# zd11024/NaviLLM

Measured on NVIDIA H100. Metric: nav_steps_per_sec, higher is better.
Workload: dtype bf16

## Files before the change

### navillm_b200/csrc/gemm_bf16.cu

```cuda
#include "nv_common.cuh"
#include "nv_fp8.cuh"
#include "nv_host.h"

namespace nv {

constexpr uint32_t GEMM_BLOCK_M = 128;
constexpr uint32_t GEMM_BLOCK_K = 64;
constexpr uint32_t GEMM_THREADS = 288;
constexpr uint32_t GEMM_CONSUMERS = 256;
constexpr uint32_t GEMM_GROUP_M = 16;

enum GemmFlags : uint32_t {
  GEMM_ADD = 1u,
  GEMM_OUT_F32 = 2u,
  GEMM_NO_GU = 4u,
};

enum { EPI_PLAIN = 0, EPI_SWIGLU = 1, EPI_DSWIGLU = 2, EPI_ROPE = 3, EPI_ATTND = 4 };

struct EpiAux {
  void* aux;
  int64_t ld_aux;
  uint32_t F;
  float* dvec;
  const int* pos;
  const __nv_bfloat16* cos_t;
  const __nv_bfloat16* sin_t;
  uint32_t rope_cols;
  const int8_t* w_exp;
};

template <uint32_t BLOCK_N, uint32_t STAGES, typename WT = __nv_bfloat16>
struct GemmSmem {
  static constexpr bool kFp8 = sizeof(WT) == 1;
  static constexpr uint32_t THREADS = kFp8 ? GEMM_THREADS + 128 : GEMM_THREADS;
  static constexpr uint32_t A_BYTES = GEMM_BLOCK_M * GEMM_BLOCK_K * 2;
  static constexpr uint32_t B_BYTES = BLOCK_N * GEMM_BLOCK_K * sizeof(WT);
  static constexpr uint32_t STAGE_BYTES = A_BYTES + B_BYTES;
  static constexpr uint32_t CVT_BYTES = kFp8 ? BLOCK_N * GEMM_BLOCK_K * 2 : 0;
  static constexpr uint32_t CVT_OFF = STAGES * STAGE_BYTES;
  static constexpr uint32_t BAR_OFF = CVT_OFF + STAGES * CVT_BYTES;
  static constexpr uint32_t DYN_BYTES = BAR_OFF + (kFp8 ? 3 : 2) * STAGES * 8 + 1024;
  static_assert(CVT_OFF % 1024 == 0, "the expanded stages are 128-byte-swizzle atoms");
  static constexpr uint32_t ACC_LD = BLOCK_N + 4;
  static_assert(GEMM_BLOCK_M * ACC_LD * 4 <= BAR_OFF, "accumulator staging reuses the stage ring");
  static_assert(DYN_BYTES <= 232448, "shared memory per block");
};

__device__ __forceinline__ void tile_coords(uint32_t tile, uint32_t num_m, uint32_t num_n, uint32_t& m_blk,
                                            uint32_t& n_blk, uint32_t group_m = GEMM_GROUP_M) {
  const uint32_t group_size = group_m * num_n;
  const uint32_t g = tile / group_size;
  const uint32_t first_m = g * group_m;
  const uint32_t gm = min(num_m - first_m, group_m);
  const uint32_t r = tile - g * group_size;
  m_blk = first_m + r % gm;
  n_blk = r / gm;
}

__device__ __forceinline__ float silu_bf16(float g) { return bf16_round(g / (1.f + __expf(-g))); }

__device__ __forceinline__ void ld_acc32(const float* p, uint32_t (&v)[32]) {
#pragma unroll
  for (uint32_t j = 0; j < 32; j += 4) {
    const uint4 x = *reinterpret_cast<const uint4*>(p + j);
    v[j] = x.x; v[j + 1] = x.y; v[j + 2] = x.z; v[j + 3] = x.w;
  }
}

template <uint32_t BLOCK_N, uint32_t STAGES, bool A_MN, bool B_MN, int EPI, typename WT = __nv_bfloat16>
__global__ void __launch_bounds__(GemmSmem<BLOCK_N, STAGES, WT>::THREADS, 1)
gemm_bf16_wgmma(const __grid_constant__ CUtensorMap tmap_a, const __grid_constant__ CUtensorMap tmap_b,
                void* __restrict__ Cout, int64_t ldc, const __nv_bfloat16* __restrict__ addend, int64_t ld_add,
                uint32_t M, uint32_t N, uint32_t K, uint32_t flags, EpiAux ea) {
  using L = GemmSmem<BLOCK_N, STAGES, WT>;
  static_assert(EPI == EPI_PLAIN || BLOCK_N == 256, "fused epilogues use the 128 x 256 tile");
  static_assert(!L::kFp8 || (EPI == EPI_PLAIN && !A_MN && !B_MN && BLOCK_N <= 128),
                "fp8 weights: plain epilogue, K-major operands, 32- or 128-wide tiles");
  extern __shared__ uint8_t smem_raw[];
  uint8_t* smem = reinterpret_cast<uint8_t*>((reinterpret_cast<uintptr_t>(smem_raw) + 1023) & ~uintptr_t(1023));
  uint8_t* smem_a = smem;
  uint8_t* smem_b = smem + STAGES * L::A_BYTES;
  uint8_t* smem_cvt = smem + L::CVT_OFF;
  uint64_t* full_bar = reinterpret_cast<uint64_t*>(smem + L::BAR_OFF);
  uint64_t* empty_bar = full_bar + STAGES;
  uint64_t* cvt_bar = empty_bar + STAGES;

  const uint32_t warp = warp_id_uniform();
  constexpr uint32_t TILE_N = (EPI == EPI_SWIGLU) ? 128u : BLOCK_N;
  const uint32_t num_m = ceil_div_u32(M, GEMM_BLOCK_M);
  const uint32_t num_n = ceil_div_u32(N, TILE_N);
  const uint32_t num_kb = ceil_div_u32(K, GEMM_BLOCK_K);
  uint32_t m_blk, n_blk;
  tile_coords(blockIdx.x, num_m, num_n, m_blk, n_blk);

  if (threadIdx.x == 0) {
    for (uint32_t i = 0; i < STAGES; ++i) {
      mbar_init(&full_bar[i], 1);
      mbar_init(&empty_bar[i], L::kFp8 ? 2 + 128 : 2);
      if constexpr (L::kFp8) mbar_init(&cvt_bar[i], 128);
    }
    fence_mbar_init();
  }
  __syncthreads();

  if (warp == 8) {
    tma_prefetch_desc(&tmap_a);
    tma_prefetch_desc(&tmap_b);
    const int32_t m0 = m_blk * GEMM_BLOCK_M;
    uint32_t stage = 0, phase = 0;
    for (uint32_t kb = 0; kb < num_kb; ++kb) {
      mbar_wait(&empty_bar[stage], phase ^ 1);
      if (elect_one()) {
        mbar_arrive_expect_tx(&full_bar[stage], L::STAGE_BYTES);
        const int32_t k0 = kb * GEMM_BLOCK_K;
        uint8_t* sa = smem_a + stage * L::A_BYTES;
        uint8_t* sb = smem_b + stage * L::B_BYTES;
        if constexpr (!A_MN) {
          tma_load_2d(sa, &tmap_a, &full_bar[stage], k0, m0);
        } else {
#pragma unroll
          for (uint32_t i = 0; i < GEMM_BLOCK_M / 64; ++i)
            tma_load_2d(sa + i * (GEMM_BLOCK_K * 128), &tmap_a, &full_bar[stage], m0 + i * 64, k0);
        }
        if constexpr (L::kFp8) {
          tma_load_2d(sb, &tmap_b, &full_bar[stage], k0, n_blk * BLOCK_N);
        } else if constexpr (!B_MN) {
          constexpr uint32_t BOX = BLOCK_N < 128 ? BLOCK_N : 128;
#pragma unroll
          for (uint32_t i = 0; i < BLOCK_N / BOX; ++i) {
            const int32_t n0 = (EPI == EPI_SWIGLU) ? (int32_t)(n_blk * 128 + i * ea.F) : (int32_t)(n_blk * BLOCK_N + i * BOX);
            tma_load_2d(sb + i * BOX * 128, &tmap_b, &full_bar[stage], k0, n0);
          }
        } else {
#pragma unroll
          for (uint32_t i = 0; i < BLOCK_N / 64; ++i)
            tma_load_2d(sb + i * (GEMM_BLOCK_K * 128), &tmap_b, &full_bar[stage], n_blk * BLOCK_N + i * 64, k0);
        }
      }
      __syncwarp();
      if (++stage == STAGES) { stage = 0; phase ^= 1; }
    }
    return;
  }

  if constexpr (L::kFp8) {
    if (warp >= 9) {
      constexpr uint32_t J = BLOCK_N * GEMM_BLOCK_K / 16 / 128;
      const uint32_t t = threadIdx.x - GEMM_THREADS;
      float scale[J];
#pragma unroll
      for (uint32_t j = 0; j < J; ++j) {
        const uint32_t n = n_blk * BLOCK_N + ((t + 128 * j) >> 2);
        scale[j] = n < N ? fp8_pow2(ea.w_exp[n]) : 1.f;
      }
      uint32_t stage = 0, phase = 0;
      for (uint32_t kb = 0; kb < num_kb; ++kb) {
        mbar_wait(&full_bar[stage], phase);
        const uint32_t src = smem_u32(smem_b + stage * L::B_BYTES);
        const uint32_t dst = smem_u32(smem_cvt + stage * L::CVT_BYTES);
#pragma unroll
        for (uint32_t j = 0; j < J; ++j) {
          const uint32_t q = t + 128 * j, row = q >> 2, c = q & 3;
          uint4 v;
          asm volatile("ld.shared.v4.b32 {%0, %1, %2, %3}, [%4];" : "=r"(v.x), "=r"(v.y), "=r"(v.z), "=r"(v.w) : "r"(src + q * 16));
          uint32_t o[8];
          fp8x4_to_bf16x4(v.x, scale[j], o[0], o[1]);
          fp8x4_to_bf16x4(v.y, scale[j], o[2], o[3]);
          fp8x4_to_bf16x4(v.z, scale[j], o[4], o[5]);
          fp8x4_to_bf16x4(v.w, scale[j], o[6], o[7]);
          sts128(dst + sw128_offset(row, 2 * c), o[0], o[1], o[2], o[3]);
          sts128(dst + sw128_offset(row, 2 * c + 1), o[4], o[5], o[6], o[7]);
        }
        fence_proxy_async_smem();
        mbar_arrive(&cvt_bar[stage]);
        mbar_arrive(&empty_bar[stage]);
        if (++stage == STAGES) { stage = 0; phase ^= 1; }
      }
      return;
    }
  }

  const uint32_t wg = warp >> 2;
  float acc[BLOCK_N / 2];
#pragma unroll
  for (uint32_t i = 0; i < BLOCK_N / 2; ++i) acc[i] = 0.f;
  {
    constexpr uint32_t A_KADV = A_MN ? (16 * 128) >> 4 : (16 * 2) >> 4;
    constexpr uint32_t B_KADV = B_MN ? (16 * 128) >> 4 : (16 * 2) >> 4;
    constexpr uint32_t A_LBO = A_MN ? GEMM_BLOCK_K * 128 : 0, B_LBO = B_MN ? GEMM_BLOCK_K * 128 : 0;
    uint32_t stage = 0, phase = 0, prev = 0;
    __builtin_assume(num_kb > 0);
    for (uint32_t kb = 0; kb < num_kb; ++kb) {
      mbar_wait(&full_bar[stage], phase);
      if constexpr (L::kFp8) mbar_wait(&cvt_bar[stage], phase);
      const uint64_t adesc = gmma_desc_sw128(smem_u32(smem_a + stage * L::A_BYTES + wg * 8192), A_LBO, 1024);
      const uint64_t bdesc = gmma_desc_sw128(smem_u32(L::kFp8 ? smem_cvt + stage * L::CVT_BYTES : smem_b + stage * L::B_BYTES),
                                             B_LBO, 1024);
      wgmma_fence();
#pragma unroll
      for (uint32_t k = 0; k < GEMM_BLOCK_K / 16; ++k)
        wgmma_ss_bf16<BLOCK_N, A_MN ? 1 : 0, B_MN ? 1 : 0>(acc, adesc + k * A_KADV, bdesc + k * B_KADV, 1u);
      wgmma_commit();
      wgmma_wait<1>();
      if (kb > 0 && (threadIdx.x & 127) == 0) mbar_arrive(&empty_bar[prev]);
      prev = stage;
      if (++stage == STAGES) { stage = 0; phase ^= 1; }
    }
    wgmma_wait<0>();
    reg_fence(acc);
  }

  float* acc_s = reinterpret_cast<float*>(smem);
  named_bar_sync(1, GEMM_CONSUMERS);
  {
    const uint32_t t = threadIdx.x & 127, lane = threadIdx.x & 31;
    const uint32_t r0 = wg * 64 + (t >> 5) * 16 + (lane >> 2);
#pragma unroll
    for (uint32_t i = 0; i < BLOCK_N / 8; ++i) {
      const uint32_t c = i * 8 + 2 * (lane & 3);
      *reinterpret_cast<float2*>(acc_s + r0 * L::ACC_LD + c) = make_float2(acc[4 * i], acc[4 * i + 1]);
      *reinterpret_cast<float2*>(acc_s + (r0 + 8) * L::ACC_LD + c) = make_float2(acc[4 * i + 2], acc[4 * i + 3]);
    }
  }
  named_bar_sync(1, GEMM_CONSUMERS);

  const uint32_t rl = threadIdx.x & 127, half = threadIdx.x >> 7;
  const uint32_t row = m_blk * GEMM_BLOCK_M + rl;
  const uint32_t col0 = n_blk * TILE_N;
  const float* arow = acc_s + rl * L::ACC_LD;
  if (row >= M) return;
  if constexpr (EPI == EPI_SWIGLU) {
    __nv_bfloat16* gu = reinterpret_cast<__nv_bfloat16*>(Cout) + static_cast<int64_t>(row) * ldc;
    __nv_bfloat16* hrow = reinterpret_cast<__nv_bfloat16*>(ea.aux) + static_cast<int64_t>(row) * ea.ld_aux;
#pragma unroll 1
    for (uint32_t c = half * 32; c < 128; c += 64) {
      uint32_t g[32], u[32];
      ld_acc32(arow + c, g);
      ld_acc32(arow + 128 + c, u);
      const uint32_t col = col0 + c;
      if (col < ea.F) {
#pragma unroll
        for (uint32_t j = 0; j < 32; j += 8) {
          uint4 og, ou, oh;
          uint32_t* pg = &og.x; uint32_t* pu = &ou.x; uint32_t* ph = &oh.x;
#pragma unroll
          for (uint32_t q = 0; q < 4; ++q) {
            pg[q] = pack_bf16x2(__uint_as_float(g[j + 2 * q]), __uint_as_float(g[j + 2 * q + 1]));
            pu[q] = pack_bf16x2(__uint_as_float(u[j + 2 * q]), __uint_as_float(u[j + 2 * q + 1]));
            ph[q] = pack_bf16x2(silu_bf16(bf16_lo(pg[q])) * bf16_lo(pu[q]), silu_bf16(bf16_hi(pg[q])) * bf16_hi(pu[q]));
          }
          if ((flags & GEMM_NO_GU) == 0) {
            *reinterpret_cast<uint4*>(gu + col + j) = og;
            *reinterpret_cast<uint4*>(gu + ea.F + col + j) = ou;
          }
          *reinterpret_cast<uint4*>(hrow + col + j) = oh;
        }
      }
    }
  } else if constexpr (EPI == EPI_DSWIGLU) {
    __nv_bfloat16* dgu = reinterpret_cast<__nv_bfloat16*>(Cout) + static_cast<int64_t>(row) * ldc;
    const __nv_bfloat16* gu = reinterpret_cast<const __nv_bfloat16*>(ea.aux) + static_cast<int64_t>(row) * ea.ld_aux;
#pragma unroll 1
    for (uint32_t c = half * 32; c < BLOCK_N; c += 64) {
      uint32_t v[32];
      ld_acc32(arow + c, v);
      const uint32_t col = col0 + c;
      if (col < ea.F) {
#pragma unroll
        for (uint32_t j = 0; j < 32; j += 8) {
          const uint4 gg = *reinterpret_cast<const uint4*>(gu + col + j);
          const uint4 uu = *reinterpret_cast<const uint4*>(gu + ea.F + col + j);
          const uint32_t* pg = &gg.x; const uint32_t* pu = &uu.x;
          uint4 og, ou;
          uint32_t* qg = &og.x; uint32_t* qu = &ou.x;
#pragma unroll
          for (uint32_t q = 0; q < 4; ++q) {
            float dg[2], du[2];
#pragma unroll
            for (uint32_t e = 0; e < 2; ++e) {
              const float d = bf16_round(__uint_as_float(v[j + 2 * q + e]));
              const float gv = e ? bf16_hi(pg[q]) : bf16_lo(pg[q]);
              const float uv = e ? bf16_hi(pu[q]) : bf16_lo(pu[q]);
              const float sg = 1.f / (1.f + __expf(-gv));
              dg[e] = d * uv * (sg * (1.f + gv * (1.f - sg)));
              du[e] = d * (gv * sg);
            }
            qg[q] = pack_bf16x2(dg[0], dg[1]);
            qu[q] = pack_bf16x2(du[0], du[1]);
          }
          *reinterpret_cast<uint4*>(dgu + col + j) = og;
          *reinterpret_cast<uint4*>(dgu + ea.F + col + j) = ou;
        }
      }
    }
  } else if constexpr (EPI == EPI_ROPE) {
    __nv_bfloat16* crow = reinterpret_cast<__nv_bfloat16*>(Cout) + static_cast<int64_t>(row) * ldc;
    const int p = ea.pos[row];
    const __nv_bfloat16* cs = ea.cos_t + static_cast<int64_t>(p) * 128;
    const __nv_bfloat16* sn = ea.sin_t + static_cast<int64_t>(p) * 128;
#pragma unroll 1
    for (uint32_t it = half; it < 4; it += 2) {
      const uint32_t hh = (it >> 1) * 128, c = (it & 1) * 32;
      uint32_t a[32], b[32];
      ld_acc32(arow + hh + c, a);
      ld_acc32(arow + hh + 64 + c, b);
      const uint32_t col = col0 + hh + c;
      if (col < N) {
        const bool rope = col < ea.rope_cols;
#pragma unroll
        for (uint32_t j = 0; j < 32; j += 8) {
          uint4 o1, o2;
          uint32_t* p1 = &o1.x; uint32_t* p2 = &o2.x;
          uint4 c1 = make_uint4(0, 0, 0, 0), s1 = c1, c2 = c1, s2 = c1;
          if (rope) {
            c1 = *reinterpret_cast<const uint4*>(cs + c + j);      s1 = *reinterpret_cast<const uint4*>(sn + c + j);
            c2 = *reinterpret_cast<const uint4*>(cs + 64 + c + j); s2 = *reinterpret_cast<const uint4*>(sn + 64 + c + j);
          }
          const uint32_t* pc1 = &c1.x; const uint32_t* ps1 = &s1.x; const uint32_t* pc2 = &c2.x; const uint32_t* ps2 = &s2.x;
#pragma unroll
          for (uint32_t q = 0; q < 4; ++q) {
            const uint32_t xa = pack_bf16x2(__uint_as_float(a[j + 2 * q]), __uint_as_float(a[j + 2 * q + 1]));
            const uint32_t xb = pack_bf16x2(__uint_as_float(b[j + 2 * q]), __uint_as_float(b[j + 2 * q + 1]));
            if (rope) {
              const float y1l = bf16_round(bf16_lo(xa) * bf16_lo(pc1[q])) + bf16_round(-bf16_lo(xb) * bf16_lo(ps1[q]));
              const float y1h = bf16_round(bf16_hi(xa) * bf16_hi(pc1[q])) + bf16_round(-bf16_hi(xb) * bf16_hi(ps1[q]));
              const float y2l = bf16_round(bf16_lo(xb) * bf16_lo(pc2[q])) + bf16_round(bf16_lo(xa) * bf16_lo(ps2[q]));
              const float y2h = bf16_round(bf16_hi(xb) * bf16_hi(pc2[q])) + bf16_round(bf16_hi(xa) * bf16_hi(ps2[q]));
              p1[q] = pack_bf16x2(y1l, y1h);
              p2[q] = pack_bf16x2(y2l, y2h);
            } else {
              p1[q] = xa;
              p2[q] = xb;
            }
          }
          *reinterpret_cast<uint4*>(crow + col + j) = o1;
          *reinterpret_cast<uint4*>(crow + col + 64 + j) = o2;
        }
      }
    }
  } else if constexpr (EPI == EPI_ATTND) {
    __nv_bfloat16* drow = reinterpret_cast<__nv_bfloat16*>(Cout) + static_cast<int64_t>(row) * ldc;
    const __nv_bfloat16* orow = reinterpret_cast<const __nv_bfloat16*>(ea.aux) + static_cast<int64_t>(row) * ea.ld_aux;
    const uint32_t hc = col0 + half * 128;
    if (hc < N) {
      float dsum = 0.f;
#pragma unroll 1
      for (uint32_t c = 0; c < 128; c += 32) {
        uint32_t v[32];
        ld_acc32(arow + half * 128 + c, v);
        const uint32_t col = hc + c;
#pragma unroll
        for (uint32_t j = 0; j < 32; j += 8) {
          uint4 o;
          o.x = pack_bf16x2(__uint_as_float(v[j + 0]), __uint_as_float(v[j + 1]));
          o.y = pack_bf16x2(__uint_as_float(v[j + 2]), __uint_as_float(v[j + 3]));
          o.z = pack_bf16x2(__uint_as_float(v[j + 4]), __uint_as_float(v[j + 5]));
          o.w = pack_bf16x2(__uint_as_float(v[j + 6]), __uint_as_float(v[j + 7]));
          const uint4 a = *reinterpret_cast<const uint4*>(orow + col + j);
          dsum += bf16_lo(o.x) * bf16_lo(a.x) + bf16_hi(o.x) * bf16_hi(a.x) + bf16_lo(o.y) * bf16_lo(a.y) + bf16_hi(o.y) * bf16_hi(a.y)
                + bf16_lo(o.z) * bf16_lo(a.z) + bf16_hi(o.z) * bf16_hi(a.z) + bf16_lo(o.w) * bf16_lo(a.w) + bf16_hi(o.w) * bf16_hi(a.w);
          *reinterpret_cast<uint4*>(drow + col + j) = o;
        }
      }
      ea.dvec[static_cast<int64_t>(hc >> 7) * M + row] = dsum;
    }
  } else {
    const bool do_add = (flags & GEMM_ADD) != 0;
    const bool out_f32 = (flags & GEMM_OUT_F32) != 0;
#pragma unroll 1
    for (uint32_t c = half * 32; c < BLOCK_N; c += 64) {
      uint32_t v[32];
      ld_acc32(arow + c, v);
      const uint32_t col = col0 + c;
      if (col >= N) break;
      if (out_f32) {
        float* dst = reinterpret_cast<float*>(Cout) + static_cast<int64_t>(row) * ldc + col;
        if (col + 32 <= N && (ldc & 3) == 0) {
#pragma unroll
          for (uint32_t j = 0; j < 32; j += 4)
            *reinterpret_cast<uint4*>(dst + j) = make_uint4(v[j], v[j + 1], v[j + 2], v[j + 3]);
        } else {
#pragma unroll
          for (uint32_t j = 0; j < 32; ++j)
            if (col + j < N) dst[j] = __uint_as_float(v[j]);
        }
      } else {
        __nv_bfloat16* dst = reinterpret_cast<__nv_bfloat16*>(Cout) + static_cast<int64_t>(row) * ldc + col;
        const __nv_bfloat16* add = do_add ? addend + static_cast<int64_t>(row) * ld_add + col : nullptr;
        if (col + 32 <= N && (ldc & 7) == 0 && (!do_add || (ld_add & 7) == 0)) {
#pragma unroll
          for (uint32_t j = 0; j < 32; j += 8) {
            uint4 o;
            o.x = pack_bf16x2(__uint_as_float(v[j + 0]), __uint_as_float(v[j + 1]));
            o.y = pack_bf16x2(__uint_as_float(v[j + 2]), __uint_as_float(v[j + 3]));
            o.z = pack_bf16x2(__uint_as_float(v[j + 4]), __uint_as_float(v[j + 5]));
            o.w = pack_bf16x2(__uint_as_float(v[j + 6]), __uint_as_float(v[j + 7]));
            if (do_add) {
              const uint4 a = *reinterpret_cast<const uint4*>(add + j);
              o.x = pack_bf16x2(bf16_lo(o.x) + bf16_lo(a.x), bf16_hi(o.x) + bf16_hi(a.x));
              o.y = pack_bf16x2(bf16_lo(o.y) + bf16_lo(a.y), bf16_hi(o.y) + bf16_hi(a.y));
              o.z = pack_bf16x2(bf16_lo(o.z) + bf16_lo(a.z), bf16_hi(o.z) + bf16_hi(a.z));
              o.w = pack_bf16x2(bf16_lo(o.w) + bf16_lo(a.w), bf16_hi(o.w) + bf16_hi(a.w));
            }
            *reinterpret_cast<uint4*>(dst + j) = o;
          }
        } else {
#pragma unroll
          for (uint32_t j = 0; j < 32; ++j) {
            if (col + j < N) {
              float x = bf16_round(__uint_as_float(v[j]));
              if (do_add) x = x + __bfloat162float(add[j]);
              dst[j] = __float2bfloat16_rn(x);
            }
          }
        }
      }
    }
  }
}

template <uint32_t BN, uint32_t ST, bool A_MN, bool B_MN, int EPI = EPI_PLAIN, typename WT = __nv_bfloat16>
static int launch_gemm(const CUtensorMap& ta, const CUtensorMap& tb, void* C, int64_t ldc, const void* addend,
                       int64_t ld_add, uint32_t M, uint32_t N, uint32_t K, uint32_t flags, cudaStream_t stream,
                       EpiAux ea = EpiAux{}) {
  using L = GemmSmem<BN, ST, WT>;
  auto kern = gemm_bf16_wgmma<BN, ST, A_MN, B_MN, EPI, WT>;
  static bool attr_set = false;
  if (!attr_set) {
    NV_CUDA(cudaFuncSetAttribute(kern, cudaFuncAttributeMaxDynamicSharedMemorySize, L::DYN_BYTES));
    attr_set = true;
  }
  const uint32_t tiles = ceil_div_u32(M, GEMM_BLOCK_M) * ceil_div_u32(N, EPI == EPI_SWIGLU ? 128u : BN);
  kern<<<tiles, L::THREADS, L::DYN_BYTES, stream>>>(ta, tb, C, ldc, reinterpret_cast<const __nv_bfloat16*>(addend), ld_add,
                                                      M, N, K, flags, ea);
  NV_LAUNCH_CHECK();
  return NV_OK;
}

constexpr uint32_t WIDE_N = 256;
constexpr uint32_t WIDE_STAGES = 4;
constexpr uint32_t WIDE_CLUSTER = 2;

struct WideSmem {
  static constexpr uint32_t A_BYTES = GEMM_BLOCK_M * GEMM_BLOCK_K * 2;
  static constexpr uint32_t B_BYTES = WIDE_N * GEMM_BLOCK_K * 2;
  static constexpr uint32_t STAGE_BYTES = A_BYTES + B_BYTES;
  static constexpr uint32_t STG_OFF = WIDE_STAGES * STAGE_BYTES;
  static constexpr uint32_t STG_BYTES = GEMM_BLOCK_M * 128 * 2;
  static constexpr uint32_t BAR_OFF = STG_OFF + STG_BYTES;
  static constexpr uint32_t DYN_BYTES = BAR_OFF + 2 * WIDE_STAGES * 8 + 1024;
  static_assert(DYN_BYTES <= 232448, "shared memory per block");
};

__device__ __forceinline__ uint32_t stg_offset(uint32_t row, uint32_t chunk) {
  return row * 256u + ((chunk ^ (row & 7u)) << 4);
}
__device__ __forceinline__ int stg_chunk(uint32_t i, uint32_t p) {
  return ((i >> 3) & 1) == p ? int(i < 16 ? i - 8 * p : i - 8 - 8 * p) : -1;
}
__device__ __forceinline__ void ld_stg32(uint32_t stg, uint32_t row, uint32_t chunk, uint32_t (&w)[16]) {
#pragma unroll
  for (uint32_t q = 0; q < 4; ++q) {
    const uint4 x = lds128(stg + stg_offset(row, chunk + q));
    w[4 * q] = x.x; w[4 * q + 1] = x.y; w[4 * q + 2] = x.z; w[4 * q + 3] = x.w;
  }
}

__device__ __forceinline__ void store_plain32(const uint32_t (&w)[16], void* Cout, int64_t ldc, const __nv_bfloat16* addend,
                                              int64_t ld_add, uint32_t row, uint32_t col, uint32_t N, bool do_add) {
  if (col >= N) return;
  __nv_bfloat16* dst = reinterpret_cast<__nv_bfloat16*>(Cout) + static_cast<int64_t>(row) * ldc + col;
  const __nv_bfloat16* add = do_add ? addend + static_cast<int64_t>(row) * ld_add + col : nullptr;
  if (col + 32 <= N && (ldc & 7) == 0 && (!do_add || (ld_add & 7) == 0)) {
#pragma unroll
    for (uint32_t j = 0; j < 4; ++j) {
      uint4 o = make_uint4(w[4 * j], w[4 * j + 1], w[4 * j + 2], w[4 * j + 3]);
      if (do_add) {
        const uint4 a = *reinterpret_cast<const uint4*>(add + 8 * j);
        o.x = pack_bf16x2(bf16_lo(o.x) + bf16_lo(a.x), bf16_hi(o.x) + bf16_hi(a.x));
        o.y = pack_bf16x2(bf16_lo(o.y) + bf16_lo(a.y), bf16_hi(o.y) + bf16_hi(a.y));
        o.z = pack_bf16x2(bf16_lo(o.z) + bf16_lo(a.z), bf16_hi(o.z) + bf16_hi(a.z));
        o.w = pack_bf16x2(bf16_lo(o.w) + bf16_lo(a.w), bf16_hi(o.w) + bf16_hi(a.w));
      }
      *reinterpret_cast<uint4*>(dst + 8 * j) = o;
    }
  } else {
#pragma unroll
    for (uint32_t j = 0; j < 32; ++j) {
      if (col + j < N) {
        float x = (j & 1) ? bf16_hi(w[j >> 1]) : bf16_lo(w[j >> 1]);
        if (do_add) x = x + __bfloat162float(add[j]);
        dst[j] = __float2bfloat16_rn(x);
      }
    }
  }
}

template <bool A_MN, bool B_MN>
__global__ void __launch_bounds__(GEMM_THREADS, 1)
gemm_bf16_wide(const __grid_constant__ CUtensorMap tmap_a, const __grid_constant__ CUtensorMap tmap_b,
               void* __restrict__ Cout, int64_t ldc, const __nv_bfloat16* __restrict__ addend, int64_t ld_add,
               uint32_t M, uint32_t N, uint32_t K, uint32_t flags) {
  using L = WideSmem;
  extern __shared__ uint8_t smem_raw[];
  uint8_t* smem = reinterpret_cast<uint8_t*>((reinterpret_cast<uintptr_t>(smem_raw) + 1023) & ~uintptr_t(1023));
  uint8_t* smem_a = smem;
  uint8_t* smem_b = smem + WIDE_STAGES * L::A_BYTES;
  const uint32_t stg = smem_u32(smem + L::STG_OFF);
  uint64_t* full_bar = reinterpret_cast<uint64_t*>(smem + L::BAR_OFF);
  uint64_t* empty_bar = full_bar + WIDE_STAGES;

  const uint32_t warp = warp_id_uniform();
  const uint32_t rank = cluster_ctarank();
  const uint32_t pair = blockIdx.x / WIDE_CLUSTER;
  const uint32_t num_m = ceil_div_u32(M, GEMM_BLOCK_M);
  const uint32_t num_mp = ceil_div_u32(num_m, WIDE_CLUSTER);
  const uint32_t num_n = ceil_div_u32(N, WIDE_N);
  const uint32_t num_kb = ceil_div_u32(K, GEMM_BLOCK_K);

  if (threadIdx.x == 0) {
    for (uint32_t i = 0; i < WIDE_STAGES; ++i) {
      mbar_init(&full_bar[i], 1);
      mbar_init(&empty_bar[i], 2 * WIDE_CLUSTER);
    }
    fence_mbar_init();
  }
  cluster_sync_all();

  uint32_t mp, n_blk;
  tile_coords(pair, num_mp, num_n, mp, n_blk, GEMM_GROUP_M / WIDE_CLUSTER);
  const uint32_t m_blk = mp * WIDE_CLUSTER + rank;

  if (warp == 8) {
    tma_prefetch_desc(&tmap_a);
    tma_prefetch_desc(&tmap_b);
    uint32_t stage = 0, phase = 0;
    {
      const int32_t m0 = m_blk * GEMM_BLOCK_M;
      for (uint32_t kb = 0; kb < num_kb; ++kb) {
        mbar_wait(&empty_bar[stage], phase ^ 1);
        if (elect_one()) {
          mbar_arrive_expect_tx(&full_bar[stage], L::STAGE_BYTES);
          const int32_t k0 = kb * GEMM_BLOCK_K;
          uint8_t* sa = smem_a + stage * L::A_BYTES;
          uint8_t* sb = smem_b + stage * L::B_BYTES;
          if constexpr (!A_MN) {
            tma_load_2d(sa, &tmap_a, &full_bar[stage], k0, m0);
          } else {
#pragma unroll
            for (uint32_t i = 0; i < GEMM_BLOCK_M / 64; ++i)
              tma_load_2d(sa + i * (GEMM_BLOCK_K * 128), &tmap_a, &full_bar[stage], m0 + i * 64, k0);
          }
          constexpr uint32_t BOXES = B_MN ? WIDE_N / 64 : 2, BOX_BYTES = L::B_BYTES / BOXES;
#pragma unroll
          for (uint32_t j = 0; j < BOXES / WIDE_CLUSTER; ++j) {
            const uint32_t i = rank * (BOXES / WIDE_CLUSTER) + j;
            int32_t c0, c1;
            if constexpr (B_MN) { c0 = n_blk * WIDE_N + i * 64; c1 = k0; }
            else { c0 = k0; c1 = n_blk * WIDE_N + i * 128; }
            tma_load_2d_multicast(sb + i * BOX_BYTES, &tmap_b, &full_bar[stage], c0, c1, (1u << WIDE_CLUSTER) - 1);
          }
        }
        __syncwarp();
        if (++stage == WIDE_STAGES) { stage = 0; phase ^= 1; }
      }
    }
  } else {
    const uint32_t wg = warp >> 2, t = threadIdx.x & 127, lane = threadIdx.x & 31;
    const uint32_t r0 = wg * 64 + (t >> 5) * 16 + (lane >> 2);
    constexpr uint32_t A_KADV = A_MN ? (16 * 128) >> 4 : (16 * 2) >> 4;
    constexpr uint32_t B_KADV = B_MN ? (16 * 128) >> 4 : (16 * 2) >> 4;
    constexpr uint32_t A_LBO = A_MN ? GEMM_BLOCK_K * 128 : 0, B_LBO = B_MN ? GEMM_BLOCK_K * 128 : 0;
    const bool do_add = (flags & GEMM_ADD) != 0;
    uint32_t stage = 0, phase = 0;
    {
      float acc[WIDE_N / 2];
#pragma unroll
      for (uint32_t i = 0; i < WIDE_N / 2; ++i) acc[i] = 0.f;
      uint32_t prev = 0;
      for (uint32_t kb = 0; kb < num_kb; ++kb) {
        mbar_wait(&full_bar[stage], phase);
        const uint64_t adesc = gmma_desc_sw128(smem_u32(smem_a + stage * L::A_BYTES + wg * 8192), A_LBO, 1024);
        const uint64_t bdesc = gmma_desc_sw128(smem_u32(smem_b + stage * L::B_BYTES), B_LBO, 1024);
        wgmma_fence();
#pragma unroll
        for (uint32_t k = 0; k < GEMM_BLOCK_K / 16; ++k)
          wgmma_ss_bf16<WIDE_N, A_MN ? 1 : 0, B_MN ? 1 : 0>(acc, adesc + k * A_KADV, bdesc + k * B_KADV, 1u);
        wgmma_commit();
        wgmma_wait<1>();
        if (kb > 0 && t == 0)
          for (uint32_t c = 0; c < WIDE_CLUSTER; ++c) mbar_arrive_cluster(&empty_bar[prev], c);
        prev = stage;
        if (++stage == WIDE_STAGES) { stage = 0; phase ^= 1; }
      }
      wgmma_wait<0>();
      reg_fence(acc);

      const uint32_t row = m_blk * GEMM_BLOCK_M + t;
      const uint32_t col0 = n_blk * WIDE_N;
#pragma unroll
      for (uint32_t p = 0; p < 2; ++p) {
        named_bar_sync(1, GEMM_CONSUMERS);
#pragma unroll
        for (uint32_t i = 0; i < WIDE_N / 8; ++i) {
          const int sc = stg_chunk(i, p);
          if (sc < 0) continue;
          sts32(stg + stg_offset(r0, sc) + 4 * (lane & 3), pack_bf16x2(acc[4 * i], acc[4 * i + 1]));
          sts32(stg + stg_offset(r0 + 8, sc) + 4 * (lane & 3), pack_bf16x2(acc[4 * i + 2], acc[4 * i + 3]));
        }
        named_bar_sync(1, GEMM_CONSUMERS);
        if (row >= M) continue;
#pragma unroll 1
          for (uint32_t h = 0; h < 2; ++h) {
            uint32_t v[16];
            ld_stg32(stg, t, 8 * h + 4 * wg, v);
            store_plain32(v, Cout, ldc, addend, ld_add, row, col0 + 128 * h + 64 * p + 32 * wg, N, do_add);
          }
      }
    }
  }
  __syncwarp();
  cluster_sync_all();
}

template <bool A_MN, bool B_MN>
static int launch_wide(const CUtensorMap& ta, const CUtensorMap& tb, void* C, int64_t ldc, const void* addend,
                       int64_t ld_add, uint32_t M, uint32_t N, uint32_t K, uint32_t flags, cudaStream_t stream) {
  auto kern = gemm_bf16_wide<A_MN, B_MN>;
  cudaLaunchConfig_t cfg = {};
  cfg.blockDim = dim3(GEMM_THREADS);
  cfg.dynamicSmemBytes = WideSmem::DYN_BYTES;
  cfg.stream = stream;
  cudaLaunchAttribute attr[1];
  attr[0].id = cudaLaunchAttributeClusterDimension;
  attr[0].val.clusterDim.x = WIDE_CLUSTER;
  attr[0].val.clusterDim.y = 1;
  attr[0].val.clusterDim.z = 1;
  cfg.attrs = attr;
  cfg.numAttrs = 1;
  static bool attr_set = false;
  if (!attr_set) {
    NV_CUDA(cudaFuncSetAttribute(kern, cudaFuncAttributeMaxDynamicSharedMemorySize, WideSmem::DYN_BYTES));
    attr_set = true;
  }
  const uint32_t pairs = ceil_div_u32(ceil_div_u32(M, GEMM_BLOCK_M), WIDE_CLUSTER) * ceil_div_u32(N, WIDE_N);
  cfg.gridDim = dim3(WIDE_CLUSTER * pairs);
  NV_CUDA(cudaLaunchKernelEx(&cfg, kern, ta, tb, C, ldc, reinterpret_cast<const __nv_bfloat16*>(addend), ld_add, M, N, K,
                             flags));
  return NV_OK;
}

static int gemm_tmaps(CUtensorMap* ta, CUtensorMap* tb, const void* A, int64_t lda, int a_mn, const void* B, int64_t ldb,
                      int b_mn, int M, int N, int K, uint32_t block_n, uint64_t b_rows) {
  int rc;
  if (!a_mn) rc = make_tmap_2d(ta, A, 2, (uint64_t)K, (uint64_t)M, (uint64_t)lda * 2, 64, GEMM_BLOCK_M);
  else       rc = make_tmap_2d(ta, A, 2, (uint64_t)M, (uint64_t)K, (uint64_t)lda * 2, 64, GEMM_BLOCK_K);
  if (rc) return rc;
  if (!b_mn) rc = make_tmap_2d(tb, B, 2, (uint64_t)K, b_rows, (uint64_t)ldb * 2, 64, block_n < 128 ? block_n : 128);
  else       rc = make_tmap_2d(tb, B, 2, (uint64_t)N, (uint64_t)K, (uint64_t)ldb * 2, 64, GEMM_BLOCK_K);
  return rc;
}

}

extern "C" int nv_gemm_bf16(const void* A, int64_t lda, int a_mn, const void* B, int64_t ldb, int b_mn, void* C,
                            int64_t ldc, const void* addend, int64_t ld_add, int M, int N, int K, unsigned flags,
                            int block_n, void* stream_) {
  using namespace nv;
  cudaStream_t stream = reinterpret_cast<cudaStream_t>(stream_);
  NV_REQUIRE(M > 0 && N > 0 && K > 0, "nv_gemm_bf16: empty problem M=%d N=%d K=%d", M, N, K);
  NV_REQUIRE(A && B && C, "nv_gemm_bf16: null operand");
  NV_REQUIRE(!(flags & GEMM_ADD) || addend, "nv_gemm_bf16: GEMM_ADD without addend");
  NV_REQUIRE(!((flags & GEMM_ADD) && (flags & GEMM_OUT_F32)), "nv_gemm_bf16: ADD with fp32 output unsupported");
  NV_REQUIRE((lda & 7) == 0 && (ldb & 7) == 0, "nv_gemm_bf16: lda/ldb must be multiples of 8 (got %lld, %lld)",
             (long long)lda, (long long)ldb);
  if (block_n == 0) {
    const long wide_tiles = ((long)(M + 127) / 128) * ((long)(N + 255) / 256);
    block_n = (wide_tiles >= sm_count() && M >= 512) ? 256 : 128;
    if (M <= 128 && !a_mn && !b_mn) block_n = N <= 4096 ? 32 : 128;
  }
  NV_REQUIRE(block_n == 32 || block_n == 128 || block_n == 256, "nv_gemm_bf16: block_n must be 32, 128 or 256");
  NV_REQUIRE(!(block_n == 32 && b_mn), "nv_gemm_bf16: block_n = 32 (skinny-M weight streaming) needs a K-major B");

  if (block_n == 256 && (flags & GEMM_OUT_F32)) block_n = 128;

  CUtensorMap ta, tb;
  int rc = gemm_tmaps(&ta, &tb, A, lda, a_mn, B, ldb, b_mn, M, N, K, (uint32_t)block_n, (uint64_t)N);
  if (rc) return rc;

  if (block_n == 256) {
    if (!a_mn && !b_mn) return launch_wide<false, false>(ta, tb, C, ldc, addend, ld_add, M, N, K, flags, stream);
    if (!a_mn && b_mn) return launch_wide<false, true>(ta, tb, C, ldc, addend, ld_add, M, N, K, flags, stream);
    if (a_mn && b_mn) return launch_wide<true, true>(ta, tb, C, ldc, addend, ld_add, M, N, K, flags, stream);
    return launch_wide<true, false>(ta, tb, C, ldc, addend, ld_add, M, N, K, flags, stream);
  }

#define NV_GEMM_CASE(BN, ST)                                                                                       \
  do {                                                                                                             \
    if (!a_mn && !b_mn) return launch_gemm<BN, ST, false, false>(ta, tb, C, ldc, addend, ld_add, M, N, K, flags, stream); \
    if (!a_mn && b_mn) return launch_gemm<BN, ST, false, true>(ta, tb, C, ldc, addend, ld_add, M, N, K, flags, stream);   \
    if (a_mn && b_mn) return launch_gemm<BN, ST, true, true>(ta, tb, C, ldc, addend, ld_add, M, N, K, flags, stream);     \
    return launch_gemm<BN, ST, true, false>(ta, tb, C, ldc, addend, ld_add, M, N, K, flags, stream);                      \
  } while (0)

  if (block_n == 32) {
    if (!a_mn) return launch_gemm<32, 10, false, false>(ta, tb, C, ldc, addend, ld_add, M, N, K, flags, stream);
    return launch_gemm<32, 10, true, false>(ta, tb, C, ldc, addend, ld_add, M, N, K, flags, stream);
  }
  NV_GEMM_CASE(128, 6);
#undef NV_GEMM_CASE
}

extern "C" int nv_gemm_fp8w_bf16(const void* A, int64_t lda, const void* Wq, int64_t ldw, const void* exps, void* C, int64_t ldc,
                                 const void* addend, int64_t ld_add, int M, int N, int K, int block_n, void* stream_) {
  using namespace nv;
  cudaStream_t stream = reinterpret_cast<cudaStream_t>(stream_);
  NV_REQUIRE(M > 0 && N > 0 && K > 0, "nv_gemm_fp8w_bf16: empty problem M=%d N=%d K=%d", M, N, K);
  NV_REQUIRE(A && Wq && exps && C, "nv_gemm_fp8w_bf16: null operand");
  NV_REQUIRE((lda & 7) == 0 && (ldw & 15) == 0,
             "nv_gemm_fp8w_bf16: lda must be a multiple of 8 and ldw (bytes) of 16 (got %lld, %lld)", (long long)lda, (long long)ldw);
  if (block_n == 0) block_n = (M <= 128 && N <= 4096) ? 32 : 128;
  NV_REQUIRE(block_n == 32 || block_n == 128, "nv_gemm_fp8w_bf16: block_n must be 0, 32 or 128 (got %d)", block_n);
  CUtensorMap ta, tb;
  int rc = make_tmap_2d(&ta, A, 2, (uint64_t)K, (uint64_t)M, (uint64_t)lda * 2, 64, GEMM_BLOCK_M);
  if (rc) return rc;
  if ((rc = make_tmap_2d(&tb, Wq, 1, (uint64_t)K, (uint64_t)N, (uint64_t)ldw, 64, (uint32_t)block_n, false)))
    return rc;
  EpiAux ea{};
  ea.w_exp = reinterpret_cast<const int8_t*>(exps);
  const uint32_t flags = addend ? GEMM_ADD : 0u;
  if (block_n == 32)
    return launch_gemm<32, 10, false, false, EPI_PLAIN, uint8_t>(ta, tb, C, ldc, addend, ld_add, M, N, K, flags, stream, ea);
  return launch_gemm<128, 5, false, false, EPI_PLAIN, uint8_t>(ta, tb, C, ldc, addend, ld_add, M, N, K, flags, stream, ea);
}

extern "C" {

int nv_gemm_swiglu_bf16(const void* x, int64_t ldx, const void* Wgu, int64_t ldw, void* gu, int64_t ldgu, void* h,
                        int64_t ldh, int M, int F, int K, int keep_gu, void* stream) {
  using namespace nv;
  NV_REQUIRE(M > 0 && F > 0 && K > 0 && (F % 128) == 0, "nv_gemm_swiglu_bf16: F must be a multiple of 128 (got %d)", F);
  NV_REQUIRE((ldx & 7) == 0 && (ldw & 7) == 0 && (ldgu & 7) == 0 && (ldh & 7) == 0, "nv_gemm_swiglu_bf16: alignment");
  CUtensorMap ta, tb;
  int rc = gemm_tmaps(&ta, &tb, x, ldx, 0, Wgu, ldw, 0, M, 2 * F, K, 256, (uint64_t)2 * F);
  if (rc) return rc;
  EpiAux ea{};
  ea.aux = h; ea.ld_aux = ldh; ea.F = (uint32_t)F;
  return launch_gemm<256, 4, false, false, EPI_SWIGLU>(ta, tb, gu, ldgu, nullptr, 0, M, F, K, keep_gu ? 0u : GEMM_NO_GU,
                                                       reinterpret_cast<cudaStream_t>(stream), ea);
}

int nv_gemm_dswiglu_bf16(const void* dx, int64_t lddx, const void* Wd, int64_t ldw, const void* gu, int64_t ldgu, void* dgu,
                         int64_t lddgu, int M, int F, int D, void* stream) {
  using namespace nv;
  NV_REQUIRE(M > 0 && F > 0 && D > 0 && (F % 32) == 0, "nv_gemm_dswiglu_bf16: F %% 32");
  NV_REQUIRE((lddx & 7) == 0 && (ldw & 7) == 0 && (ldgu & 7) == 0 && (lddgu & 7) == 0, "nv_gemm_dswiglu_bf16: alignment");
  CUtensorMap ta, tb;
  int rc = gemm_tmaps(&ta, &tb, dx, lddx, 0, Wd, ldw, 1, M, F, D, 256, (uint64_t)F);
  if (rc) return rc;
  EpiAux ea{};
  ea.aux = const_cast<void*>(gu); ea.ld_aux = ldgu; ea.F = (uint32_t)F;
  return launch_gemm<256, 4, false, true, EPI_DSWIGLU>(ta, tb, dgu, lddgu, nullptr, 0, M, F, D, 0u,
                                                       reinterpret_cast<cudaStream_t>(stream), ea);
}

int nv_gemm_attnd_bf16(const void* dy, int64_t lddy, const void* Wo, int64_t ldw, const void* o, int64_t ldo, void* dout,
                       int64_t lddo, float* dvec, int M, int D, int Dout, void* stream) {
  using namespace nv;
  NV_REQUIRE(M > 0 && D > 0 && Dout > 0 && (D % 128) == 0 && o && dvec, "nv_gemm_attnd_bf16: D %% 128 and O / dvec required");
  NV_REQUIRE((lddy & 7) == 0 && (ldw & 7) == 0 && (ldo & 7) == 0 && (lddo & 7) == 0, "nv_gemm_attnd_bf16: alignment");
  CUtensorMap ta, tb;
  int rc = gemm_tmaps(&ta, &tb, dy, lddy, 0, Wo, ldw, 1, M, D, Dout, 256, (uint64_t)D);
  if (rc) return rc;
  EpiAux ea{};
  ea.aux = const_cast<void*>(o); ea.ld_aux = ldo; ea.dvec = dvec;
  return launch_gemm<256, 4, false, true, EPI_ATTND>(ta, tb, dout, lddo, nullptr, 0, M, D, Dout, 0u,
                                                     reinterpret_cast<cudaStream_t>(stream), ea);
}

int nv_gemm_rope_bf16(const void* x, int64_t ldx, const void* W, int64_t ldw, void* out, int64_t ldo, const int* pos,
                      const void* cos_t, const void* sin_t, int M, int N, int K, int rope_cols, void* stream) {
  using namespace nv;
  NV_REQUIRE(M > 0 && N > 0 && K > 0 && (N % 128) == 0 && (rope_cols % 128) == 0, "nv_gemm_rope_bf16: head alignment");
  NV_REQUIRE((ldx & 7) == 0 && (ldw & 7) == 0 && (ldo & 7) == 0, "nv_gemm_rope_bf16: alignment");
  CUtensorMap ta, tb;
  int rc = gemm_tmaps(&ta, &tb, x, ldx, 0, W, ldw, 0, M, N, K, 256, (uint64_t)N);
  if (rc) return rc;
  EpiAux ea{};
  ea.pos = pos; ea.cos_t = reinterpret_cast<const __nv_bfloat16*>(cos_t); ea.sin_t = reinterpret_cast<const __nv_bfloat16*>(sin_t);
  ea.rope_cols = (uint32_t)rope_cols;
  return launch_gemm<256, 4, false, false, EPI_ROPE>(ta, tb, out, ldo, nullptr, 0, M, N, K, 0u,
                                                     reinterpret_cast<cudaStream_t>(stream), ea);
}

}
```

### navillm_b200/csrc/nv_common.cuh

```cuda
#pragma once

#include <cuda.h>
#include <cuda_bf16.h>
#include <cuda_runtime.h>
#include <stdint.h>
#include <stdio.h>

#include "nv_wgmma.cuh"

namespace nv {

__device__ __forceinline__ uint32_t smem_u32(const void* p) {
  return static_cast<uint32_t>(__cvta_generic_to_shared(p));
}
__device__ __forceinline__ uint32_t lane_id() {
  uint32_t l;
  asm volatile("mov.u32 %0, %%laneid;" : "=r"(l));
  return l;
}
__host__ __device__ constexpr uint32_t ceil_div_u32(uint32_t a, uint32_t b) { return (a + b - 1) / b; }

__device__ __forceinline__ uint32_t pack_bf16x2(float a, float b) {
  __nv_bfloat162 v = __floats2bfloat162_rn(a, b);
  return *reinterpret_cast<uint32_t*>(&v);
}
__device__ __forceinline__ float bf16_lo(uint32_t v) { return __uint_as_float(v << 16); }
__device__ __forceinline__ float bf16_hi(uint32_t v) { return __uint_as_float(v & 0xffff0000u); }
__device__ __forceinline__ float bf16_round(float x) { return __bfloat162float(__float2bfloat16_rn(x)); }

__device__ __forceinline__ void griddep_wait() { asm volatile("griddepcontrol.wait;" ::: "memory"); }
__device__ __forceinline__ void griddep_launch() { asm volatile("griddepcontrol.launch_dependents;" ::: "memory"); }

__device__ __forceinline__ void sts128(uint32_t saddr, uint32_t a, uint32_t b, uint32_t c, uint32_t d) {
  asm volatile("st.shared.v4.b32 [%0], {%1, %2, %3, %4};" ::"r"(saddr), "r"(a), "r"(b), "r"(c), "r"(d) : "memory");
}
__device__ __forceinline__ void sts32(uint32_t saddr, uint32_t a) {
  asm volatile("st.shared.b32 [%0], %1;" ::"r"(saddr), "r"(a) : "memory");
}
__device__ __forceinline__ uint4 lds128(uint32_t saddr) {
  uint4 v;
  asm volatile("ld.shared.v4.b32 {%0, %1, %2, %3}, [%4];" : "=r"(v.x), "=r"(v.y), "=r"(v.z), "=r"(v.w) : "r"(saddr) : "memory");
  return v;
}
__device__ __forceinline__ uint2 lds64(uint32_t saddr) {
  uint2 v;
  asm volatile("ld.shared.v2.b32 {%0, %1}, [%2];" : "=r"(v.x), "=r"(v.y) : "r"(saddr) : "memory");
  return v;
}

__device__ __forceinline__ void mbar_init(uint64_t* bar, uint32_t count) {
  asm volatile("mbarrier.init.shared::cta.b64 [%0], %1;" ::"r"(smem_u32(bar)), "r"(count) : "memory");
}
__device__ __forceinline__ void fence_mbar_init() {
  asm volatile("fence.mbarrier_init.release.cluster;" ::: "memory");
}
__device__ __forceinline__ void mbar_arrive(uint64_t* bar) {
  asm volatile("mbarrier.arrive.shared::cta.b64 _, [%0];" ::"r"(smem_u32(bar)) : "memory");
}
__device__ __forceinline__ void mbar_arrive_expect_tx(uint64_t* bar, uint32_t bytes) {
  asm volatile("mbarrier.arrive.expect_tx.shared::cta.b64 _, [%0], %1;" ::"r"(smem_u32(bar)), "r"(bytes)
               : "memory");
}
__device__ __forceinline__ bool mbar_try_wait(uint64_t* bar, uint32_t parity) {
  uint32_t ok;
  asm volatile(
      "{\n\t.reg .pred p;\n\t"
      "mbarrier.try_wait.parity.shared::cta.b64 p, [%1], %2;\n\t"
      "selp.u32 %0, 1, 0, p;\n\t}"
      : "=r"(ok)
      : "r"(smem_u32(bar)), "r"(parity)
      : "memory");
  return ok != 0;
}
#ifndef NV_MBAR_TIMEOUT_CYCLES
#define NV_MBAR_TIMEOUT_CYCLES (4000000000ll)
#endif
__device__ __forceinline__ void mbar_wait(uint64_t* bar, uint32_t parity) {
  if (mbar_try_wait(bar, parity)) return;
  const long long t0 = clock64();
  uint32_t spins = 0;
  while (!mbar_try_wait(bar, parity)) {
    if ((++spins & 255u) == 0 && clock64() - t0 > NV_MBAR_TIMEOUT_CYCLES) {
#ifdef NV_MBAR_TIMEOUT_REPORT
      printf("navillm_b200: mbarrier timeout block (%d,%d) thread %d bar@%u parity %u\n", (int)blockIdx.x,
             (int)blockIdx.y, (int)threadIdx.x, smem_u32(bar), parity);
#endif
      __trap();
    }
  }
}

__device__ __forceinline__ void fence_proxy_async_smem() {
  asm volatile("fence.proxy.async.shared::cta;" ::: "memory");
}

__device__ __forceinline__ void tma_prefetch_desc(const CUtensorMap* m) {
  asm volatile("prefetch.tensormap [%0];" ::"l"(reinterpret_cast<uint64_t>(m)) : "memory");
}
__device__ __forceinline__ void tma_load_2d(void* smem_dst, const CUtensorMap* m, uint64_t* bar, int32_t c0,
                                            int32_t c1) {
  asm volatile(
      "cp.async.bulk.tensor.2d.shared::cluster.global.mbarrier::complete_tx::bytes [%0], [%1, {%3, %4}], [%2];"
      ::"r"(smem_u32(smem_dst)), "l"(reinterpret_cast<uint64_t>(m)), "r"(smem_u32(bar)), "r"(c0), "r"(c1)
      : "memory");
}
__device__ __forceinline__ void tma_load_2d_multicast(void* smem_dst, const CUtensorMap* m, uint64_t* bar, int32_t c0,
                                                      int32_t c1, uint16_t cta_mask) {
  asm volatile(
      "cp.async.bulk.tensor.2d.shared::cluster.global.mbarrier::complete_tx::bytes.multicast::cluster"
      " [%0], [%1, {%3, %4}], [%2], %5;"
      ::"r"(smem_u32(smem_dst)), "l"(reinterpret_cast<uint64_t>(m)), "r"(smem_u32(bar)), "r"(c0), "r"(c1), "h"(cta_mask)
      : "memory");
}
__device__ __forceinline__ void tma_load_3d(void* smem_dst, const CUtensorMap* m, uint64_t* bar, int32_t c0,
                                            int32_t c1, int32_t c2) {
  asm volatile(
      "cp.async.bulk.tensor.3d.shared::cluster.global.mbarrier::complete_tx::bytes [%0], [%1, {%3, %4, %5}], [%2];"
      ::"r"(smem_u32(smem_dst)), "l"(reinterpret_cast<uint64_t>(m)), "r"(smem_u32(bar)), "r"(c0), "r"(c1), "r"(c2)
      : "memory");
}
__device__ __forceinline__ void tma_store_2d(const CUtensorMap* m, const void* smem_src, int32_t c0, int32_t c1) {
  asm volatile("cp.async.bulk.tensor.2d.global.shared::cta.bulk_group [%0, {%2, %3}], [%1];" ::"l"(
                   reinterpret_cast<uint64_t>(m)),
               "r"(smem_u32(smem_src)), "r"(c0), "r"(c1)
               : "memory");
}
__device__ __forceinline__ void tma_store_commit() { asm volatile("cp.async.bulk.commit_group;" ::: "memory"); }
template <int N>
__device__ __forceinline__ void tma_store_wait_read() {
  asm volatile("cp.async.bulk.wait_group.read %0;" ::"n"(N) : "memory");
}
template <int N>
__device__ __forceinline__ void tma_store_wait_all() {
  asm volatile("cp.async.bulk.wait_group %0;" ::"n"(N) : "memory");
}

__device__ __forceinline__ void wgmma_fence() { asm volatile("wgmma.fence.sync.aligned;" ::: "memory"); }
__device__ __forceinline__ void wgmma_commit() { asm volatile("wgmma.commit_group.sync.aligned;" ::: "memory"); }
template <int N>
__device__ __forceinline__ void wgmma_wait() {
  asm volatile("wgmma.wait_group.sync.aligned %0;" ::"n"(N) : "memory");
}
template <int R>
__device__ __forceinline__ void reg_fence(float (&d)[R]) {
#pragma unroll
  for (int i = 0; i < R; ++i) asm volatile("" : "+f"(d[i])::"memory");
}

__device__ __forceinline__ bool elect_one() {
  uint32_t pred;
  asm volatile("{\n\t.reg .pred e;\n\telect.sync _|e, 0xffffffff;\n\tselp.u32 %0, 1, 0, e;\n\t}" : "=r"(pred));
  return pred != 0;
}
__device__ __forceinline__ uint32_t warp_id_uniform() { return __shfl_sync(0xffffffffu, threadIdx.x >> 5, 0); }

__device__ __forceinline__ void named_bar_sync(uint32_t id, uint32_t count) {
  asm volatile("bar.sync %0, %1;" ::"r"(id), "r"(count) : "memory");
}

__device__ __forceinline__ void cluster_sync_all() {
  asm volatile("barrier.cluster.arrive.release.aligned;\n\tbarrier.cluster.wait.acquire.aligned;" ::: "memory");
}
__device__ __forceinline__ uint32_t cluster_ctarank() {
  uint32_t r;
  asm volatile("mov.u32 %0, %%cluster_ctarank;" : "=r"(r));
  return r;
}
__device__ __forceinline__ void mbar_arrive_cluster(uint64_t* bar, uint32_t cta) {
  asm volatile(
      "{\n\t.reg .b32 ra;\n\t"
      "mapa.shared::cluster.u32 ra, %0, %1;\n\t"
      "mbarrier.arrive.shared::cluster.b64 _, [ra];\n\t}"
      ::"r"(smem_u32(bar)), "r"(cta)
      : "memory");
}
__device__ __forceinline__ void dsmem_add_f32(uint32_t saddr, uint32_t cta, float v) {
  asm volatile(
      "{\n\t.reg .b32 ra;\n\t.reg .f32 x;\n\t"
      "mapa.shared::cluster.u32 ra, %0, %1;\n\t"
      "ld.shared::cluster.f32 x, [ra];\n\t"
      "add.f32 x, x, %2;\n\t"
      "st.shared::cluster.f32 [ra], x;\n\t}"
      ::"r"(saddr), "r"(cta), "f"(v)
      : "memory");
}

__device__ __forceinline__ uint64_t gmma_desc_sw128(uint32_t smem_addr, uint32_t lbo_bytes, uint32_t sbo_bytes) {
  uint64_t d = 0;
  d |= static_cast<uint64_t>((smem_addr >> 4) & 0x3FFFu);
  d |= static_cast<uint64_t>((lbo_bytes >> 4) & 0x3FFFu) << 16;
  d |= static_cast<uint64_t>((sbo_bytes >> 4) & 0x3FFFu) << 32;
  d |= static_cast<uint64_t>(1) << 62;
  return d;
}

__device__ __forceinline__ uint32_t sw128_offset(uint32_t row, uint32_t chunk) {
  return row * 128u + ((chunk ^ (row & 7u)) << 4);
}

}
```

Measured before the change: 22.23.

## Move fused SwiGLU/dSwiGLU/RoPE/attn-backward epilogues onto the clustered wide GEMM kernel

Removes the fused-epilogue variants from the simple 128x256 wgmma kernel and reimplements them in the clustered wide GEMM kernel. The new epilogues stage outputs in recycled pipeline smem slots with swizzled layouts and write them with TMA stores through per-epilogue tensor maps, and they also TMA-prefetch the auxiliary operands (gu, o). The goal is to give the fused MLP and attention-backward GEMMs the faster wide mainloop and to replace strided per-thread global stores and loads with bulk TMA traffic. This adds complexity in smem slot reuse and barrier handling, and there is risk of correctness issues in the swizzled epilogue indexing.

```diff
diff --git a/navillm_b200/csrc/gemm_bf16.cu b/navillm_b200/csrc/gemm_bf16.cu
--- a/navillm_b200/csrc/gemm_bf16.cu
+++ b/navillm_b200/csrc/gemm_bf16.cu
@@ -19,8 +19,6 @@
 enum { EPI_PLAIN = 0, EPI_SWIGLU = 1, EPI_DSWIGLU = 2, EPI_ROPE = 3, EPI_ATTND = 4 };
 
 struct EpiAux {
-  void* aux;
-  int64_t ld_aux;
   uint32_t F;
   float* dvec;
   const int* pos;
@@ -68,15 +66,14 @@
   }
 }
 
-template <uint32_t BLOCK_N, uint32_t STAGES, bool A_MN, bool B_MN, int EPI, typename WT = __nv_bfloat16>
+template <uint32_t BLOCK_N, uint32_t STAGES, bool A_MN, bool B_MN, typename WT = __nv_bfloat16>
 __global__ void __launch_bounds__(GemmSmem<BLOCK_N, STAGES, WT>::THREADS, 1)
 gemm_bf16_wgmma(const __grid_constant__ CUtensorMap tmap_a, const __grid_constant__ CUtensorMap tmap_b,
                 void* __restrict__ Cout, int64_t ldc, const __nv_bfloat16* __restrict__ addend, int64_t ld_add,
                 uint32_t M, uint32_t N, uint32_t K, uint32_t flags, EpiAux ea) {
   using L = GemmSmem<BLOCK_N, STAGES, WT>;
-  static_assert(EPI == EPI_PLAIN || BLOCK_N == 256, "fused epilogues use the 128 x 256 tile");
-  static_assert(!L::kFp8 || (EPI == EPI_PLAIN && !A_MN && !B_MN && BLOCK_N <= 128),
-                "fp8 weights: plain epilogue, K-major operands, 32- or 128-wide tiles");
+  static_assert(BLOCK_N <= 128, "the 128 x 256 tile is gemm_bf16_wide");
+  static_assert(!L::kFp8 || (!A_MN && !B_MN), "fp8 weights: K-major operands");
   extern __shared__ uint8_t smem_raw[];
   uint8_t* smem = reinterpret_cast<uint8_t*>((reinterpret_cast<uintptr_t>(smem_raw) + 1023) & ~uintptr_t(1023));
   uint8_t* smem_a = smem;
@@ -87,9 +84,8 @@
   uint64_t* cvt_bar = empty_bar + STAGES;
 
   const uint32_t warp = warp_id_uniform();
-  constexpr uint32_t TILE_N = (EPI == EPI_SWIGLU) ? 128u : BLOCK_N;
   const uint32_t num_m = ceil_div_u32(M, GEMM_BLOCK_M);
-  const uint32_t num_n = ceil_div_u32(N, TILE_N);
+  const uint32_t num_n = ceil_div_u32(N, BLOCK_N);
   const uint32_t num_kb = ceil_div_u32(K, GEMM_BLOCK_K);
   uint32_t m_blk, n_blk;
   tile_coords(blockIdx.x, num_m, num_n, m_blk, n_blk);
@@ -129,8 +125,7 @@
           constexpr uint32_t BOX = BLOCK_N < 128 ? BLOCK_N : 128;
 #pragma unroll
           for (uint32_t i = 0; i < BLOCK_N / BOX; ++i) {
-            const int32_t n0 = (EPI == EPI_SWIGLU) ? (int32_t)(n_blk * 128 + i * ea.F) : (int32_t)(n_blk * BLOCK_N + i * BOX);
-            tma_load_2d(sb + i * BOX * 128, &tmap_b, &full_bar[stage], k0, n0);
+            tma_load_2d(sb + i * BOX * 128, &tmap_b, &full_bar[stage], k0, n_blk * BLOCK_N + i * BOX);
           }
         } else {
 #pragma unroll
@@ -227,129 +222,32 @@
 
   const uint32_t rl = threadIdx.x & 127, half = threadIdx.x >> 7;
   const uint32_t row = m_blk * GEMM_BLOCK_M + rl;
-  const uint32_t col0 = n_blk * TILE_N;
+  const uint32_t col0 = n_blk * BLOCK_N;
   const float* arow = acc_s + rl * L::ACC_LD;
   if (row >= M) return;
-  if constexpr (EPI == EPI_SWIGLU) {
-    __nv_bfloat16* gu = reinterpret_cast<__nv_bfloat16*>(Cout) + static_cast<int64_t>(row) * ldc;
-    __nv_bfloat16* hrow = reinterpret_cast<__nv_bfloat16*>(ea.aux) + static_cast<int64_t>(row) * ea.ld_aux;
+  const bool do_add = (flags & GEMM_ADD) != 0;
+  const bool out_f32 = (flags & GEMM_OUT_F32) != 0;
 #pragma unroll 1
-    for (uint32_t c = half * 32; c < 128; c += 64) {
-      uint32_t g[32], u[32];
-      ld_acc32(arow + c, g);
-      ld_acc32(arow + 128 + c, u);
-      const uint32_t col = col0 + c;
-      if (col < ea.F) {
-#pragma unroll
-        for (uint32_t j = 0; j < 32; j += 8) {
-          uint4 og, ou, oh;
-          uint32_t* pg = &og.x; uint32_t* pu = &ou.x; uint32_t* ph = &oh.x;
-#pragma unroll
-          for (uint32_t q = 0; q < 4; ++q) {
-            pg[q] = pack_bf16x2(__uint_as_float(g[j + 2 * q]), __uint_as_float(g[j + 2 * q + 1]));
-            pu[q] = pack_bf16x2(__uint_as_float(u[j + 2 * q]), __uint_as_float(u[j + 2 * q + 1]));
-            ph[q] = pack_bf16x2(silu_bf16(bf16_lo(pg[q])) * bf16_lo(pu[q]), silu_bf16(bf16_hi(pg[q])) * bf16_hi(pu[q]));
-          }
-          if ((flags & GEMM_NO_GU) == 0) {
-            *reinterpret_cast<uint4*>(gu + col + j) = og;
-            *reinterpret_cast<uint4*>(gu + ea.F + col + j) = ou;
-          }
-          *reinterpret_cast<uint4*>(hrow + col + j) = oh;
-        }
-      }
-    }
-  } else if constexpr (EPI == EPI_DSWIGLU) {
-    __nv_bfloat16* dgu = reinterpret_cast<__nv_bfloat16*>(Cout) + static_cast<int64_t>(row) * ldc;
-    const __nv_bfloat16* gu = reinterpret_cast<const __nv_bfloat16*>(ea.aux) + static_cast<int64_t>(row) * ea.ld_aux;
-#pragma unroll 1
-    for (uint32_t c = half * 32; c < BLOCK_N; c += 64) {
-      uint32_t v[32];
-      ld_acc32(arow + c, v);
-      const uint32_t col = col0 + c;
-      if (col < ea.F) {
-#pragma unroll
-        for (uint32_t j = 0; j < 32; j += 8) {
-          const uint4 gg = *reinterpret_cast<const uint4*>(gu + col + j);
-          const uint4 uu = *reinterpret_cast<const uint4*>(gu + ea.F + col + j);
-          const uint32_t* pg = &gg.x; const uint32_t* pu = &uu.x;
-          uint4 og, ou;
-          uint32_t* qg = &og.x; uint32_t* qu = &ou.x;
-#pragma unroll
-          for (uint32_t q = 0; q < 4; ++q) {
-            float dg[2], du[2];
-#pragma unroll
-            for (uint32_t e = 0; e < 2; ++e) {
-              const float d = bf16_round(__uint_as_float(v[j + 2 * q + e]));
-              const float gv = e ? bf16_hi(pg[q]) : bf16_lo(pg[q]);
-              const float uv = e ? bf16_hi(pu[q]) : bf16_lo(pu[q]);
-              const float sg = 1.f / (1.f + __expf(-gv));
-              dg[e] = d * uv * (sg * (1.f + gv * (1.f - sg)));
-              du[e] = d * (gv * sg);
-            }
-            qg[q] = pack_bf16x2(dg[0], dg[1]);
-            qu[q] = pack_bf16x2(du[0], du[1]);
-          }
-          *reinterpret_cast<uint4*>(dgu + col + j) = og;
-          *reinterpret_cast<uint4*>(dgu + ea.F + col + j) = ou;
-        }
-      }
-    }
-  } else if constexpr (EPI == EPI_ROPE) {
-    __nv_bfloat16* crow = reinterpret_cast<__nv_bfloat16*>(Cout) + static_cast<int64_t>(row) * ldc;
-    const int p = ea.pos[row];
-    const __nv_bfloat16* cs = ea.cos_t + static_cast<int64_t>(p) * 128;
-    const __nv_bfloat16* sn = ea.sin_t + static_cast<int64_t>(p) * 128;
-#pragma unroll 1
-    for (uint32_t it = half; it < 4; it += 2) {
-      const uint32_t hh = (it >> 1) * 128, c = (it & 1) * 32;
-      uint32_t a[32], b[32];
-      ld_acc32(arow + hh + c, a);
-      ld_acc32(arow + hh + 64 + c, b);
-      const uint32_t col = col0 + hh + c;
-      if (col < N) {
-        const bool rope = col < ea.rope_cols;
-#pragma unroll
-        for (uint32_t j = 0; j < 32; j += 8) {
-          uint4 o1, o2;
-          uint32_t* p1 = &o1.x; uint32_t* p2 = &o2.x;
-          uint4 c1 = make_uint4(0, 0, 0, 0), s1 = c1, c2 = c1, s2 = c1;
-          if (rope) {
-            c1 = *reinterpret_cast<const uint4*>(cs + c + j);      s1 = *reinterpret_cast<const uint4*>(sn + c + j);
-            c2 = *reinterpret_cast<const uint4*>(cs + 64 + c + j); s2 = *reinterpret_cast<const uint4*>(sn + 64 + c + j);
-          }
-          const uint32_t* pc1 = &c1.x; const uint32_t* ps1 = &s1.x; const uint32_t* pc2 = &c2.x; const uint32_t* ps2 = &s2.x;
-#pragma unroll
-          for (uint32_t q = 0; q < 4; ++q) {
-            const uint32_t xa = pack_bf16x2(__uint_as_float(a[j + 2 * q]), __uint_as_float(a[j + 2 * q + 1]));
-            const uint32_t xb = pack_bf16x2(__uint_as_float(b[j + 2 * q]), __uint_as_float(b[j + 2 * q + 1]));
-            if (rope) {
-              const float y1l = bf16_round(bf16_lo(xa) * bf16_lo(pc1[q])) + bf16_round(-bf16_lo(xb) * bf16_lo(ps1[q]));
-              const float y1h = bf16_round(bf16_hi(xa) * bf16_hi(pc1[q])) + bf16_round(-bf16_hi(xb) * bf16_hi(ps1[q]));
-              const float y2l = bf16_round(bf16_lo(xb) * bf16_lo(pc2[q])) + bf16_round(bf16_lo(xa) * bf16_lo(ps2[q]));
-              const float y2h = bf16_round(bf16_hi(xb) * bf16_hi(pc2[q])) + bf16_round(bf16_hi(xa) * bf16_hi(ps2[q]));
-              p1[q] = pack_bf16x2(y1l, y1h);
-              p2[q] = pack_bf16x2(y2l, y2h);
-            } else {
-              p1[q] = xa;
-              p2[q] = xb;
-            }
-          }
-          *reinterpret_cast<uint4*>(crow + col + j) = o1;
-          *reinterpret_cast<uint4*>(crow + col + 64 + j) = o2;
-        }
-      }
-    }
-  } else if constexpr (EPI == EPI_ATTND) {
-    __nv_bfloat16* drow = reinterpret_cast<__nv_bfloat16*>(Cout) + static_cast<int64_t>(row) * ldc;
-    const __nv_bfloat16* orow = reinterpret_cast<const __nv_bfloat16*>(ea.aux) + static_cast<int64_t>(row) * ea.ld_aux;
-    const uint32_t hc = col0 + half * 128;
-    if (hc < N) {
-      float dsum = 0.f;
-#pragma unroll 1
-      for (uint32_t c = 0; c < 128; c += 32) {
-        uint32_t v[32];
-        ld_acc32(arow + half * 128 + c, v);
-        const uint32_t col = hc + c;
+  for (uint32_t c = half * 32; c < BLOCK_N; c += 64) {
+    uint32_t v[32];
+    ld_acc32(arow + c, v);
+    const uint32_t col = col0 + c;
+    if (col >= N) break;
+    if (out_f32) {
+      float* dst = reinterpret_cast<float*>(Cout) + static_cast<int64_t>(row) * ldc + col;
+      if (col + 32 <= N && (ldc & 3) == 0) {
+#pragma unroll
+        for (uint32_t j = 0; j < 32; j += 4)
+          *reinterpret_cast<uint4*>(dst + j) = make_uint4(v[j], v[j + 1], v[j + 2], v[j + 3]);
+      } else {
+#pragma unroll
+        for (uint32_t j = 0; j < 32; ++j)
+          if (col + j < N) dst[j] = __uint_as_float(v[j]);
+      }
+    } else {
+      __nv_bfloat16* dst = reinterpret_cast<__nv_bfloat16*>(Cout) + static_cast<int64_t>(row) * ldc + col;
+      const __nv_bfloat16* add = do_add ? addend + static_cast<int64_t>(row) * ld_add + col : nullptr;
+      if (col + 32 <= N && (ldc & 7) == 0 && (!do_add || (ld_add & 7) == 0)) {
 #pragma unroll
         for (uint32_t j = 0; j < 32; j += 8) {
           uint4 o;
@@ -357,81 +255,41 @@
           o.y = pack_bf16x2(__uint_as_float(v[j + 2]), __uint_as_float(v[j + 3]));
           o.z = pack_bf16x2(__uint_as_float(v[j + 4]), __uint_as_float(v[j + 5]));
           o.w = pack_bf16x2(__uint_as_float(v[j + 6]), __uint_as_float(v[j + 7]));
-          const uint4 a = *reinterpret_cast<const uint4*>(orow + col + j);
-          dsum += bf16_lo(o.x) * bf16_lo(a.x) + bf16_hi(o.x) * bf16_hi(a.x) + bf16_lo(o.y) * bf16_lo(a.y) + bf16_hi(o.y) * bf16_hi(a.y)
-                + bf16_lo(o.z) * bf16_lo(a.z) + bf16_hi(o.z) * bf16_hi(a.z) + bf16_lo(o.w) * bf16_lo(a.w) + bf16_hi(o.w) * bf16_hi(a.w);
-          *reinterpret_cast<uint4*>(drow + col + j) = o;
-        }
-      }
-      ea.dvec[static_cast<int64_t>(hc >> 7) * M + row] = dsum;
-    }
-  } else {
-    const bool do_add = (flags & GEMM_ADD) != 0;
-    const bool out_f32 = (flags & GEMM_OUT_F32) != 0;
-#pragma unroll 1
-    for (uint32_t c = half * 32; c < BLOCK_N; c += 64) {
-      uint32_t v[32];
-      ld_acc32(arow + c, v);
-      const uint32_t col = col0 + c;
-      if (col >= N) break;
-      if (out_f32) {
-        float* dst = reinterpret_cast<float*>(Cout) + static_cast<int64_t>(row) * ldc + col;
-        if (col + 32 <= N && (ldc & 3) == 0) {
-#pragma unroll
-          for (uint32_t j = 0; j < 32; j += 4)
-            *reinterpret_cast<uint4*>(dst + j) = make_uint4(v[j], v[j + 1], v[j + 2], v[j + 3]);
-        } else {
-#pragma unroll
-          for (uint32_t j = 0; j < 32; ++j)
-            if (col + j < N) dst[j] = __uint_as_float(v[j]);
+          if (do_add) {
+            const uint4 a = *reinterpret_cast<const uint4*>(add + j);
+            o.x = pack_bf16x2(bf16_lo(o.x) + bf16_lo(a.x), bf16_hi(o.x) + bf16_hi(a.x));
+            o.y = pack_bf16x2(bf16_lo(o.y) + bf16_lo(a.y), bf16_hi(o.y) + bf16_hi(a.y));
+            o.z = pack_bf16x2(bf16_lo(o.z) + bf16_lo(a.z), bf16_hi(o.z) + bf16_hi(a.z));
+            o.w = pack_bf16x2(bf16_lo(o.w) + bf16_lo(a.w), bf16_hi(o.w) + bf16_hi(a.w));
+          }
+          *reinterpret_cast<uint4*>(dst + j) = o;
         }
       } else {
-        __nv_bfloat16* dst = reinterpret_cast<__nv_bfloat16*>(Cout) + static_cast<int64_t>(row) * ldc + col;
-        const __nv_bfloat16* add = do_add ? addend + static_cast<int64_t>(row) * ld_add + col : nullptr;
-        if (col + 32 <= N && (ldc & 7) == 0 && (!do_add || (ld_add & 7) == 0)) {
-#pragma unroll
-          for (uint32_t j = 0; j < 32; j += 8) {
-            uint4 o;
-            o.x = pack_bf16x2(__uint_as_float(v[j + 0]), __uint_as_float(v[j + 1]));
-            o.y = pack_bf16x2(__uint_as_float(v[j + 2]), __uint_as_float(v[j + 3]));
-            o.z = pack_bf16x2(__uint_as_float(v[j + 4]), __uint_as_float(v[j + 5]));
-            o.w = pack_bf16x2(__uint_as_float(v[j + 6]), __uint_as_float(v[j + 7]));
-            if (do_add) {
-              const uint4 a = *reinterpret_cast<const uint4*>(add + j);
-              o.x = pack_bf16x2(bf16_lo(o.x) + bf16_lo(a.x), bf16_hi(o.x) + bf16_hi(a.x));
-              o.y = pack_bf16x2(bf16_lo(o.y) + bf16_lo(a.y), bf16_hi(o.y) + bf16_hi(a.y));
-              o.z = pack_bf16x2(bf16_lo(o.z) + bf16_lo(a.z), bf16_hi(o.z) + bf16_hi(a.z));
-              o.w = pack_bf16x2(bf16_lo(o.w) + bf16_lo(a.w), bf16_hi(o.w) + bf16_hi(a.w));
-            }
-            *reinterpret_cast<uint4*>(dst + j) = o;
+#pragma unroll
+        for (uint32_t j = 0; j < 32; ++j) {
+          if (col + j < N) {
+            float x = bf16_round(__uint_as_float(v[j]));
+            if (do_add) x = x + __bfloat162float(add[j]);
+            dst[j] = __float2bfloat16_rn(x);
           }
-        } else {
-#pragma unroll
-          for (uint32_t j = 0; j < 32; ++j) {
-            if (col + j < N) {
-              float x = bf16_round(__uint_as_float(v[j]));
-              if (do_add) x = x + __bfloat162float(add[j]);
-              dst[j] = __float2bfloat16_rn(x);
-            }
-          }
-        }
-      }
-    }
-  }
-}
-
-template <uint32_t BN, uint32_t ST, bool A_MN, bool B_MN, int EPI = EPI_PLAIN, typename WT = __nv_bfloat16>
+        }
+      }
+    }
+  }
+}
+
+template <uint32_t BN, uint32_t ST, bool A_MN, bool B_MN, typename WT = __nv_bfloat16>
 static int launch_gemm(const CUtensorMap& ta, const CUtensorMap& tb, void* C, int64_t ldc, const void* addend,
                        int64_t ld_add, uint32_t M, uint32_t N, uint32_t K, uint32_t flags, cudaStream_t stream,
                        EpiAux ea = EpiAux{}) {
   using L = GemmSmem<BN, ST, WT>;
-  auto kern = gemm_bf16_wgmma<BN, ST, A_MN, B_MN, EPI, WT>;
+  auto kern = gemm_bf16_wgmma<BN, ST, A_MN, B_MN, WT>;
   static bool attr_set = false;
   if (!attr_set) {
     NV_CUDA(cudaFuncSetAttribute(kern, cudaFuncAttributeMaxDynamicSharedMemorySize, L::DYN_BYTES));
     attr_set = true;
   }
-  const uint32_t tiles = ceil_div_u32(M, GEMM_BLOCK_M) * ceil_div_u32(N, EPI == EPI_SWIGLU ? 128u : BN);
+  const uint32_t tiles = ceil_div_u32(M, GEMM_BLOCK_M) * ceil_div_u32(N, BN);
   kern<<<tiles, L::THREADS, L::DYN_BYTES, stream>>>(ta, tb, C, ldc, reinterpret_cast<const __nv_bfloat16*>(addend), ld_add,
                                                       M, N, K, flags, ea);
   NV_LAUNCH_CHECK();
@@ -449,7 +307,7 @@
   static constexpr uint32_t STG_OFF = WIDE_STAGES * STAGE_BYTES;
   static constexpr uint32_t STG_BYTES = GEMM_BLOCK_M * 128 * 2;
   static constexpr uint32_t BAR_OFF = STG_OFF + STG_BYTES;
-  static constexpr uint32_t DYN_BYTES = BAR_OFF + 2 * WIDE_STAGES * 8 + 1024;
+  static constexpr uint32_t DYN_BYTES = BAR_OFF + (2 * WIDE_STAGES + 1) * 8 + 1024;
   static_assert(DYN_BYTES <= 232448, "shared memory per block");
 };
 
@@ -497,12 +355,32 @@
   }
 }
 
-template <bool A_MN, bool B_MN>
+constexpr uint32_t EPI_BOX_BYTES = GEMM_BLOCK_M * 128;
+
+struct EpiMaps {
+  CUtensorMap m[4];
+};
+
+__device__ __forceinline__ uint8_t* epi_slot(uint8_t* smem, uint32_t num_kb, uint32_t v) {
+  const uint32_t s = (num_kb + v / 3) % WIDE_STAGES, j = v % 3;
+  return j == 0 ? smem + s * WideSmem::A_BYTES
+                : smem + WIDE_STAGES * WideSmem::A_BYTES + s * WideSmem::B_BYTES + (j - 1) * EPI_BOX_BYTES;
+}
+__device__ __forceinline__ uint32_t frag_offset(uint32_t r, uint32_t i, uint32_t lane) {
+  return sw128_offset(r, i & 7) + 4 * (lane & 3);
+}
+
+template <bool A_MN, bool B_MN, int EPI>
 __global__ void __launch_bounds__(GEMM_THREADS, 1)
 gemm_bf16_wide(const __grid_constant__ CUtensorMap tmap_a, const __grid_constant__ CUtensorMap tmap_b,
-               void* __restrict__ Cout, int64_t ldc, const __nv_bfloat16* __restrict__ addend, int64_t ld_add,
-               uint32_t M, uint32_t N, uint32_t K, uint32_t flags) {
+               const __grid_constant__ EpiMaps em, void* __restrict__ Cout, int64_t ldc,
+               const __nv_bfloat16* __restrict__ addend, int64_t ld_add, uint32_t M, uint32_t N, uint32_t K,
+               uint32_t flags, EpiAux ea) {
   using L = WideSmem;
+  static_assert(EPI == EPI_PLAIN || (!A_MN && B_MN == (EPI == EPI_DSWIGLU || EPI == EPI_ATTND)),
+                "fused epilogues: the operand forms of their entry points");
+  constexpr uint32_t TILE_N = EPI == EPI_SWIGLU ? 128u : WIDE_N;
+  constexpr uint32_t PRE_BOXES = EPI == EPI_DSWIGLU ? 8 : EPI == EPI_ATTND ? 4 : 0;
   extern __shared__ uint8_t smem_raw[];
   uint8_t* smem = reinterpret_cast<uint8_t*>((reinterpret_cast<uintptr_t>(smem_raw) + 1023) & ~uintptr_t(1023));
   uint8_t* smem_a = smem;
@@ -510,13 +388,14 @@
   const uint32_t stg = smem_u32(smem + L::STG_OFF);
   uint64_t* full_bar = reinterpret_cast<uint64_t*>(smem + L::BAR_OFF);
   uint64_t* empty_bar = full_bar + WIDE_STAGES;
+  uint64_t* epi_full = empty_bar + WIDE_STAGES;
 
   const uint32_t warp = warp_id_uniform();
   const uint32_t rank = cluster_ctarank();
   const uint32_t pair = blockIdx.x / WIDE_CLUSTER;
   const uint32_t num_m = ceil_div_u32(M, GEMM_BLOCK_M);
   const uint32_t num_mp = ceil_div_u32(num_m, WIDE_CLUSTER);
-  const uint32_t num_n = ceil_div_u32(N, WIDE_N);
+  const uint32_t num_n = ceil_div_u32(N, TILE_N);
   const uint32_t num_kb = ceil_div_u32(K, GEMM_BLOCK_K);
 
   if (threadIdx.x == 0) {
@@ -524,6 +403,7 @@
       mbar_init(&full_bar[i], 1);
       mbar_init(&empty_bar[i], 2 * WIDE_CLUSTER);
     }
+    mbar_init(epi_full, 1);
     fence_mbar_init();
   }
   cluster_sync_all();
@@ -531,39 +411,55 @@
   uint32_t mp, n_blk;
   tile_coords(pair, num_mp, num_n, mp, n_blk, GEMM_GROUP_M / WIDE_CLUSTER);
   const uint32_t m_blk = mp * WIDE_CLUSTER + rank;
+  const int32_t m0 = m_blk * GEMM_BLOCK_M;
+  const uint32_t col0 = n_blk * TILE_N;
 
   if (warp == 8) {
     tma_prefetch_desc(&tmap_a);
     tma_prefetch_desc(&tmap_b);
     uint32_t stage = 0, phase = 0;
-    {
-      const int32_t m0 = m_blk * GEMM_BLOCK_M;
-      for (uint32_t kb = 0; kb < num_kb; ++kb) {
-        mbar_wait(&empty_bar[stage], phase ^ 1);
-        if (elect_one()) {
-          mbar_arrive_expect_tx(&full_bar[stage], L::STAGE_BYTES);
-          const int32_t k0 = kb * GEMM_BLOCK_K;
-          uint8_t* sa = smem_a + stage * L::A_BYTES;
-          uint8_t* sb = smem_b + stage * L::B_BYTES;
-          if constexpr (!A_MN) {
-            tma_load_2d(sa, &tmap_a, &full_bar[stage], k0, m0);
-          } else {
-#pragma unroll
-            for (uint32_t i = 0; i < GEMM_BLOCK_M / 64; ++i)
-              tma_load_2d(sa + i * (GEMM_BLOCK_K * 128), &tmap_a, &full_bar[stage], m0 + i * 64, k0);
+    for (uint32_t kb = 0; kb < num_kb; ++kb) {
+      mbar_wait(&empty_bar[stage], phase ^ 1);
+      if (elect_one()) {
+        mbar_arrive_expect_tx(&full_bar[stage], L::STAGE_BYTES);
+        const int32_t k0 = kb * GEMM_BLOCK_K;
+        uint8_t* sa = smem_a + stage * L::A_BYTES;
+        uint8_t* sb = smem_b + stage * L::B_BYTES;
+        if constexpr (!A_MN) {
+          tma_load_2d(sa, &tmap_a, &full_bar[stage], k0, m0);
+        } else {
+#pragma unroll
+          for (uint32_t i = 0; i < GEMM_BLOCK_M / 64; ++i)
+            tma_load_2d(sa + i * (GEMM_BLOCK_K * 128), &tmap_a, &full_bar[stage], m0 + i * 64, k0);
+        }
+        constexpr uint32_t BOXES = B_MN ? WIDE_N / 64 : 2, BOX_BYTES = L::B_BYTES / BOXES;
+#pragma unroll
+        for (uint32_t j = 0; j < BOXES / WIDE_CLUSTER; ++j) {
+          const uint32_t i = rank * (BOXES / WIDE_CLUSTER) + j;
+          int32_t c0, c1;
+          if constexpr (B_MN) { c0 = n_blk * WIDE_N + i * 64; c1 = k0; }
+          else { c0 = k0; c1 = EPI == EPI_SWIGLU ? col0 + i * ea.F : n_blk * WIDE_N + i * 128; }
+          tma_load_2d_multicast(sb + i * BOX_BYTES, &tmap_b, &full_bar[stage], c0, c1, (1u << WIDE_CLUSTER) - 1);
+        }
+      }
+      __syncwarp();
+      if (++stage == WIDE_STAGES) { stage = 0; phase ^= 1; }
+    }
+    if constexpr (PRE_BOXES > 0) {
+      if (m_blk < num_m) {
+        if (elect_one()) mbar_arrive_expect_tx(epi_full, PRE_BOXES * EPI_BOX_BYTES);
+        __syncwarp();
+#pragma unroll
+        for (uint32_t v0 = 0; v0 < PRE_BOXES; v0 += 3) {
+          mbar_wait(&empty_bar[stage], phase ^ 1);
+          if (elect_one()) {
+#pragma unroll
+            for (uint32_t v = v0; v < v0 + 3 && v < PRE_BOXES; ++v)
+              tma_load_2d(epi_slot(smem, num_kb, v), &em.m[2 + v / 4], epi_full, col0 + 64 * (v % 4), m0);
           }
-          constexpr uint32_t BOXES = B_MN ? WIDE_N / 64 : 2, BOX_BYTES = L::B_BYTES / BOXES;
-#pragma unroll
-          for (uint32_t j = 0; j < BOXES / WIDE_CLUSTER; ++j) {
-            const uint32_t i = rank * (BOXES / WIDE_CLUSTER) + j;
-            int32_t c0, c1;
-            if constexpr (B_MN) { c0 = n_blk * WIDE_N + i * 64; c1 = k0; }
-            else { c0 = k0; c1 = n_blk * WIDE_N + i * 128; }
-            tma_load_2d_multicast(sb + i * BOX_BYTES, &tmap_b, &full_bar[stage], c0, c1, (1u << WIDE_CLUSTER) - 1);
-          }
-        }
-        __syncwarp();
-        if (++stage == WIDE_STAGES) { stage = 0; phase ^= 1; }
+          __syncwarp();
+          if (++stage == WIDE_STAGES) { stage = 0; phase ^= 1; }
+        }
       }
     }
   } else {
@@ -572,13 +468,13 @@
     constexpr uint32_t A_KADV = A_MN ? (16 * 128) >> 4 : (16 * 2) >> 4;
     constexpr uint32_t B_KADV = B_MN ? (16 * 128) >> 4 : (16 * 2) >> 4;
     constexpr uint32_t A_LBO = A_MN ? GEMM_BLOCK_K * 128 : 0, B_LBO = B_MN ? GEMM_BLOCK_K * 128 : 0;
-    const bool do_add = (flags & GEMM_ADD) != 0;
     uint32_t stage = 0, phase = 0;
     {
       float acc[WIDE_N / 2];
 #pragma unroll
       for (uint32_t i = 0; i < WIDE_N / 2; ++i) acc[i] = 0.f;
       uint32_t prev = 0;
+      __builtin_assume(num_kb > 0);
       for (uint32_t kb = 0; kb < num_kb; ++kb) {
         mbar_wait(&full_bar[stage], phase);
         const uint64_t adesc = gmma_desc_sw128(smem_u32(smem_a + stage * L::A_BYTES + wg * 8192), A_LBO, 1024);
@@ -597,26 +493,153 @@
       wgmma_wait<0>();
       reg_fence(acc);
 
-      const uint32_t row = m_blk * GEMM_BLOCK_M + t;
-      const uint32_t col0 = n_blk * WIDE_N;
-#pragma unroll
-      for (uint32_t p = 0; p < 2; ++p) {
-        named_bar_sync(1, GEMM_CONSUMERS);
-#pragma unroll
-        for (uint32_t i = 0; i < WIDE_N / 8; ++i) {
-          const int sc = stg_chunk(i, p);
-          if (sc < 0) continue;
-          sts32(stg + stg_offset(r0, sc) + 4 * (lane & 3), pack_bf16x2(acc[4 * i], acc[4 * i + 1]));
-          sts32(stg + stg_offset(r0 + 8, sc) + 4 * (lane & 3), pack_bf16x2(acc[4 * i + 2], acc[4 * i + 3]));
-        }
-        named_bar_sync(1, GEMM_CONSUMERS);
-        if (row >= M) continue;
+      if constexpr (EPI == EPI_PLAIN) {
+        const bool do_add = (flags & GEMM_ADD) != 0;
+        const uint32_t row = m_blk * GEMM_BLOCK_M + t;
+#pragma unroll
+        for (uint32_t p = 0; p < 2; ++p) {
+          named_bar_sync(1, GEMM_CONSUMERS);
+#pragma unroll
+          for (uint32_t i = 0; i < WIDE_N / 8; ++i) {
+            const int sc = stg_chunk(i, p);
+            if (sc < 0) continue;
+            sts32(stg + stg_offset(r0, sc) + 4 * (lane & 3), pack_bf16x2(acc[4 * i], acc[4 * i + 1]));
+            sts32(stg + stg_offset(r0 + 8, sc) + 4 * (lane & 3), pack_bf16x2(acc[4 * i + 2], acc[4 * i + 3]));
+          }
+          named_bar_sync(1, GEMM_CONSUMERS);
+          if (row >= M) continue;
 #pragma unroll 1
           for (uint32_t h = 0; h < 2; ++h) {
             uint32_t v[16];
             ld_stg32(stg, t, 8 * h + 4 * wg, v);
             store_plain32(v, Cout, ldc, addend, ld_add, row, col0 + 128 * h + 64 * p + 32 * wg, N, do_add);
           }
+        }
+      } else {
+        named_bar_sync(1, GEMM_CONSUMERS);
+        if (m_blk < num_m) {
+          uint8_t* slot[8];
+#pragma unroll
+          for (uint32_t v = 0; v < 8; ++v) slot[v] = epi_slot(smem, num_kb, v);
+          constexpr uint32_t OUT_BOXES = EPI == EPI_SWIGLU ? 6 : EPI == EPI_DSWIGLU ? 8 : 4;
+          constexpr uint32_t OUT_SLOT0 = EPI == EPI_ATTND ? 4 : 0;
+          if constexpr (EPI == EPI_SWIGLU) {
+#pragma unroll
+            for (uint32_t i = 0; i < 16; ++i) {
+#pragma unroll
+              for (uint32_t h = 0; h < 2; ++h) {
+                const uint32_t g = pack_bf16x2(acc[4 * i + 2 * h], acc[4 * i + 2 * h + 1]);
+                const uint32_t u = pack_bf16x2(acc[4 * (i + 16) + 2 * h], acc[4 * (i + 16) + 2 * h + 1]);
+                const uint32_t off = frag_offset(r0 + 8 * h, i, lane);
+                sts32(smem_u32(slot[i / 8]) + off, g);
+                sts32(smem_u32(slot[2 + i / 8]) + off, u);
+                sts32(smem_u32(slot[4 + i / 8]) + off,
+                      pack_bf16x2(silu_bf16(bf16_lo(g)) * bf16_lo(u), silu_bf16(bf16_hi(g)) * bf16_hi(u)));
+              }
+            }
+          } else if constexpr (EPI == EPI_DSWIGLU) {
+            mbar_wait(epi_full, 0);
+#pragma unroll
+            for (uint32_t i = 0; i < 32; ++i) {
+#pragma unroll
+              for (uint32_t h = 0; h < 2; ++h) {
+                const uint32_t off = frag_offset(r0 + 8 * h, i, lane);
+                const uint32_t ga = smem_u32(slot[i / 8]) + off, ua = smem_u32(slot[4 + i / 8]) + off;
+                const uint32_t gp = lds32(ga), up = lds32(ua);
+                float dg[2], du[2];
+#pragma unroll
+                for (uint32_t e = 0; e < 2; ++e) {
+                  const float d = bf16_round(acc[4 * i + 2 * h + e]);
+                  const float gv = e ? bf16_hi(gp) : bf16_lo(gp);
+                  const float uv = e ? bf16_hi(up) : bf16_lo(up);
+                  const float sg = 1.f / (1.f + __expf(-gv));
+                  dg[e] = d * uv * (sg * (1.f + gv * (1.f - sg)));
+                  du[e] = d * (gv * sg);
+                }
+                sts32(ga, pack_bf16x2(dg[0], dg[1]));
+                sts32(ua, pack_bf16x2(du[0], du[1]));
+              }
+            }
+          } else if constexpr (EPI == EPI_ROPE) {
+            const bool rope0 = col0 < ea.rope_cols, rope1 = col0 + 128 < ea.rope_cols;
+            int p[2];
+#pragma unroll
+            for (uint32_t h = 0; h < 2; ++h) p[h] = m0 + r0 + 8 * h < M ? ea.pos[m0 + r0 + 8 * h] : 0;
+#pragma unroll
+            for (uint32_t i = 0; i < 8; ++i) {
+#pragma unroll
+              for (uint32_t h = 0; h < 2; ++h) {
+                const uint32_t c = 8 * i + 2 * (lane & 3), off = frag_offset(r0 + 8 * h, i, lane);
+                uint32_t c1 = 0, s1 = 0, c2 = 0, s2 = 0;
+                if (rope0) {
+                  const int64_t b = static_cast<int64_t>(p[h]) * 128 + c;
+                  c1 = *reinterpret_cast<const uint32_t*>(ea.cos_t + b);
+                  s1 = *reinterpret_cast<const uint32_t*>(ea.sin_t + b);
+                  c2 = *reinterpret_cast<const uint32_t*>(ea.cos_t + b + 64);
+                  s2 = *reinterpret_cast<const uint32_t*>(ea.sin_t + b + 64);
+                }
+#pragma unroll
+                for (uint32_t hd = 0; hd < 2; ++hd) {
+                  const uint32_t ia = 16 * hd + i, ib = ia + 8;
+                  const uint32_t xa = pack_bf16x2(acc[4 * ia + 2 * h], acc[4 * ia + 2 * h + 1]);
+                  const uint32_t xb = pack_bf16x2(acc[4 * ib + 2 * h], acc[4 * ib + 2 * h + 1]);
+                  uint32_t o1 = xa, o2 = xb;
+                  if (hd ? rope1 : rope0) {
+                    const float y1l = bf16_round(bf16_lo(xa) * bf16_lo(c1)) + bf16_round(-bf16_lo(xb) * bf16_lo(s1));
+                    const float y1h = bf16_round(bf16_hi(xa) * bf16_hi(c1)) + bf16_round(-bf16_hi(xb) * bf16_hi(s1));
+                    const float y2l = bf16_round(bf16_lo(xb) * bf16_lo(c2)) + bf16_round(bf16_lo(xa) * bf16_lo(s2));
+                    const float y2h = bf16_round(bf16_hi(xb) * bf16_hi(c2)) + bf16_round(bf16_hi(xa) * bf16_hi(s2));
+                    o1 = pack_bf16x2(y1l, y1h);
+                    o2 = pack_bf16x2(y2l, y2h);
+                  }
+                  sts32(smem_u32(slot[2 * hd]) + off, o1);
+                  sts32(smem_u32(slot[2 * hd + 1]) + off, o2);
+                }
+              }
+            }
+          } else {
+#pragma unroll
+            for (uint32_t i = 0; i < 32; ++i) {
+#pragma unroll
+              for (uint32_t h = 0; h < 2; ++h)
+                sts32(smem_u32(slot[4 + i / 8]) + frag_offset(r0 + 8 * h, i, lane),
+                      pack_bf16x2(acc[4 * i + 2 * h], acc[4 * i + 2 * h + 1]));
+            }
+          }
+          fence_proxy_async_smem();
+          named_bar_sync(1, GEMM_CONSUMERS);
+          if (threadIdx.x == 0) {
+            const uint32_t ncols = EPI == EPI_SWIGLU || EPI == EPI_DSWIGLU ? ea.F : N;
+#pragma unroll
+            for (uint32_t b = 0; b < OUT_BOXES; ++b) {
+              const uint32_t map = EPI == EPI_SWIGLU ? b / 2 : EPI == EPI_DSWIGLU ? b / 4 : 0;
+              const uint32_t col = col0 + 64 * (EPI == EPI_SWIGLU ? b % 2 : b % 4);
+              if (EPI == EPI_SWIGLU && map < 2 && (flags & GEMM_NO_GU)) continue;
+              if (col < ncols) tma_store_2d(&em.m[map], slot[OUT_SLOT0 + b], col, m0);
+            }
+            tma_store_commit();
+          }
+          if constexpr (EPI == EPI_ATTND) {
+            mbar_wait(epi_full, 0);
+            const uint32_t hc = col0 + wg * 128;
+            if (hc < N && m0 + t < M) {
+              float dsum = 0.f;
+#pragma unroll
+              for (uint32_t c = 0; c < 128; c += 32) {
+#pragma unroll
+                for (uint32_t j = 0; j < 32; j += 8) {
+                  const uint32_t bb = (c + j) / 64, off = sw128_offset(t, ((c + j) % 64) / 8);
+                  const uint4 o = lds128(smem_u32(wg ? slot[6 + bb] : slot[4 + bb]) + off);
+                  const uint4 a = lds128(smem_u32(wg ? slot[2 + bb] : slot[bb]) + off);
+                  dsum += bf16_lo(o.x) * bf16_lo(a.x) + bf16_hi(o.x) * bf16_hi(a.x) + bf16_lo(o.y) * bf16_lo(a.y) + bf16_hi(o.y) * bf16_hi(a.y)
+                        + bf16_lo(o.z) * bf16_lo(a.z) + bf16_hi(o.z) * bf16_hi(a.z) + bf16_lo(o.w) * bf16_lo(a.w) + bf16_hi(o.w) * bf16_hi(a.w);
+                }
+              }
+              ea.dvec[static_cast<int64_t>(hc >> 7) * M + m0 + t] = dsum;
+            }
+          }
+          if (threadIdx.x == 0) tma_store_wait_read<0>();
+        }
       }
     }
   }
@@ -624,10 +647,11 @@
   cluster_sync_all();
 }
 
-template <bool A_MN, bool B_MN>
+template <bool A_MN, bool B_MN, int EPI = EPI_PLAIN>
 static int launch_wide(const CUtensorMap& ta, const CUtensorMap& tb, void* C, int64_t ldc, const void* addend,
-                       int64_t ld_add, uint32_t M, uint32_t N, uint32_t K, uint32_t flags, cudaStream_t stream) {
-  auto kern = gemm_bf16_wide<A_MN, B_MN>;
+                       int64_t ld_add, uint32_t M, uint32_t N, uint32_t K, uint32_t flags, cudaStream_t stream,
+                       const EpiMaps& em = EpiMaps{}, EpiAux ea = EpiAux{}) {
+  auto kern = gemm_bf16_wide<A_MN, B_MN, EPI>;
   cudaLaunchConfig_t cfg = {};
   cfg.blockDim = dim3(GEMM_THREADS);
   cfg.dynamicSmemBytes = WideSmem::DYN_BYTES;
@@ -644,10 +668,11 @@
     NV_CUDA(cudaFuncSetAttribute(kern, cudaFuncAttributeMaxDynamicSharedMemorySize, WideSmem::DYN_BYTES));
     attr_set = true;
   }
-  const uint32_t pairs = ceil_div_u32(ceil_div_u32(M, GEMM_BLOCK_M), WIDE_CLUSTER) * ceil_div_u32(N, WIDE_N);
+  const uint32_t pairs = ceil_div_u32(ceil_div_u32(M, GEMM_BLOCK_M), WIDE_CLUSTER) *
+                         ceil_div_u32(N, EPI == EPI_SWIGLU ? 128u : WIDE_N);
   cfg.gridDim = dim3(WIDE_CLUSTER * pairs);
-  NV_CUDA(cudaLaunchKernelEx(&cfg, kern, ta, tb, C, ldc, reinterpret_cast<const __nv_bfloat16*>(addend), ld_add, M, N, K,
-                             flags));
+  NV_CUDA(cudaLaunchKernelEx(&cfg, kern, ta, tb, em, C, ldc, reinterpret_cast<const __nv_bfloat16*>(addend), ld_add, M,
+                             N, K, flags, ea));
   return NV_OK;
 }
 
@@ -731,8 +756,8 @@
   ea.w_exp = reinterpret_cast<const int8_t*>(exps);
   const uint32_t flags = addend ? GEMM_ADD : 0u;
   if (block_n == 32)
-    return launch_gemm<32, 10, false, false, EPI_PLAIN, uint8_t>(ta, tb, C, ldc, addend, ld_add, M, N, K, flags, stream, ea);
-  return launch_gemm<128, 5, false, false, EPI_PLAIN, uint8_t>(ta, tb, C, ldc, addend, ld_add, M, N, K, flags, stream, ea);
+    return launch_gemm<32, 10, false, false, uint8_t>(ta, tb, C, ldc, addend, ld_add, M, N, K, flags, stream, ea);
+  return launch_gemm<128, 5, false, false, uint8_t>(ta, tb, C, ldc, addend, ld_add, M, N, K, flags, stream, ea);
 }
 
 extern "C" {
@@ -745,10 +770,18 @@
   CUtensorMap ta, tb;
   int rc = gemm_tmaps(&ta, &tb, x, ldx, 0, Wgu, ldw, 0, M, 2 * F, K, 256, (uint64_t)2 * F);
   if (rc) return rc;
+  EpiMaps em{};
+  if (keep_gu) {
+    if ((rc = make_tmap_2d(&em.m[0], gu, 2, (uint64_t)F, (uint64_t)M, (uint64_t)ldgu * 2, 64, GEMM_BLOCK_M))) return rc;
+    if ((rc = make_tmap_2d(&em.m[1], static_cast<__nv_bfloat16*>(gu) + F, 2, (uint64_t)F, (uint64_t)M, (uint64_t)ldgu * 2, 64,
+                           GEMM_BLOCK_M)))
+      return rc;
+  }
+  if ((rc = make_tmap_2d(&em.m[2], h, 2, (uint64_t)F, (uint64_t)M, (uint64_t)ldh * 2, 64, GEMM_BLOCK_M))) return rc;
   EpiAux ea{};
-  ea.aux = h; ea.ld_aux = ldh; ea.F = (uint32_t)F;
-  return launch_gemm<256, 4, false, false, EPI_SWIGLU>(ta, tb, gu, ldgu, nullptr, 0, M, F, K, keep_gu ? 0u : GEMM_NO_GU,
-                                                       reinterpret_cast<cudaStream_t>(stream), ea);
+  ea.F = (uint32_t)F;
+  return launch_wide<false, false, EPI_SWIGLU>(ta, tb, gu, ldgu, nullptr, 0, M, F, K, keep_gu ? 0u : GEMM_NO_GU,
+                                               reinterpret_cast<cudaStream_t>(stream), em, ea);
 }
 
 int nv_gemm_dswiglu_bf16(const void* dx, int64_t lddx, const void* Wd, int64_t ldw, const void* gu, int64_t ldgu, void* dgu,
@@ -759,10 +792,17 @@
   CUtensorMap ta, tb;
   int rc = gemm_tmaps(&ta, &tb, dx, lddx, 0, Wd, ldw, 1, M, F, D, 256, (uint64_t)F);
   if (rc) return rc;
+  EpiMaps em{};
+  const __nv_bfloat16* halves[4] = {static_cast<const __nv_bfloat16*>(dgu), static_cast<const __nv_bfloat16*>(dgu) + F,
+                                    static_cast<const __nv_bfloat16*>(gu), static_cast<const __nv_bfloat16*>(gu) + F};
+  for (int i = 0; i < 4; ++i)
+    if ((rc = make_tmap_2d(&em.m[i], halves[i], 2, (uint64_t)F, (uint64_t)M, (uint64_t)(i < 2 ? lddgu : ldgu) * 2, 64,
+                           GEMM_BLOCK_M)))
+      return rc;
   EpiAux ea{};
-  ea.aux = const_cast<void*>(gu); ea.ld_aux = ldgu; ea.F = (uint32_t)F;
-  return launch_gemm<256, 4, false, true, EPI_DSWIGLU>(ta, tb, dgu, lddgu, nullptr, 0, M, F, D, 0u,
-                                                       reinterpret_cast<cudaStream_t>(stream), ea);
+  ea.F = (uint32_t)F;
+  return launch_wide<false, true, EPI_DSWIGLU>(ta, tb, dgu, lddgu, nullptr, 0, M, F, D, 0u,
+                                               reinterpret_cast<cudaStream_t>(stream), em, ea);
 }
 
 int nv_gemm_attnd_bf16(const void* dy, int64_t lddy, const void* Wo, int64_t ldw, const void* o, int64_t ldo, void* dout,
@@ -773,10 +813,13 @@
   CUtensorMap ta, tb;
   int rc = gemm_tmaps(&ta, &tb, dy, lddy, 0, Wo, ldw, 1, M, D, Dout, 256, (uint64_t)D);
   if (rc) return rc;
+  EpiMaps em{};
+  if ((rc = make_tmap_2d(&em.m[0], dout, 2, (uint64_t)D, (uint64_t)M, (uint64_t)lddo * 2, 64, GEMM_BLOCK_M))) return rc;
+  if ((rc = make_tmap_2d(&em.m[2], o, 2, (uint64_t)D, (uint64_t)M, (uint64_t)ldo * 2, 64, GEMM_BLOCK_M))) return rc;
   EpiAux ea{};
-  ea.aux = const_cast<void*>(o); ea.ld_aux = ldo; ea.dvec = dvec;
-  return launch_gemm<256, 4, false, true, EPI_ATTND>(ta, tb, dout, lddo, nullptr, 0, M, D, Dout, 0u,
-                                                     reinterpret_cast<cudaStream_t>(stream), ea);
+  ea.dvec = dvec;
+  return launch_wide<false, true, EPI_ATTND>(ta, tb, dout, lddo, nullptr, 0, M, D, Dout, 0u,
+                                             reinterpret_cast<cudaStream_t>(stream), em, ea);
 }
 
 int nv_gemm_rope_bf16(const void* x, int64_t ldx, const void* W, int64_t ldw, void* out, int64_t ldo, const int* pos,
@@ -787,11 +830,13 @@
   CUtensorMap ta, tb;
   int rc = gemm_tmaps(&ta, &tb, x, ldx, 0, W, ldw, 0, M, N, K, 256, (uint64_t)N);
   if (rc) return rc;
+  EpiMaps em{};
+  if ((rc = make_tmap_2d(&em.m[0], out, 2, (uint64_t)N, (uint64_t)M, (uint64_t)ldo * 2, 64, GEMM_BLOCK_M))) return rc;
   EpiAux ea{};
   ea.pos = pos; ea.cos_t = reinterpret_cast<const __nv_bfloat16*>(cos_t); ea.sin_t = reinterpret_cast<const __nv_bfloat16*>(sin_t);
   ea.rope_cols = (uint32_t)rope_cols;
-  return launch_gemm<256, 4, false, false, EPI_ROPE>(ta, tb, out, ldo, nullptr, 0, M, N, K, 0u,
-                                                     reinterpret_cast<cudaStream_t>(stream), ea);
-}
-
-}
+  return launch_wide<false, false, EPI_ROPE>(ta, tb, out, ldo, nullptr, 0, M, N, K, 0u,
+                                             reinterpret_cast<cudaStream_t>(stream), em, ea);
+}
+
+}
diff --git a/navillm_b200/csrc/nv_common.cuh b/navillm_b200/csrc/nv_common.cuh
--- a/navillm_b200/csrc/nv_common.cuh
+++ b/navillm_b200/csrc/nv_common.cuh
@@ -40,6 +40,11 @@
 __device__ __forceinline__ uint4 lds128(uint32_t saddr) {
   uint4 v;
   asm volatile("ld.shared.v4.b32 {%0, %1, %2, %3}, [%4];" : "=r"(v.x), "=r"(v.y), "=r"(v.z), "=r"(v.w) : "r"(saddr) : "memory");
+  return v;
+}
+__device__ __forceinline__ uint32_t lds32(uint32_t saddr) {
+  uint32_t v;
+  asm volatile("ld.shared.b32 %0, [%1];" : "=r"(v) : "r"(saddr) : "memory");
   return v;
 }
 __device__ __forceinline__ uint2 lds64(uint32_t saddr) {
```

Result: faster. 23.28, median of 6 (+4.7%).
